# real-stanford/dgdm

Measured on AMD Instinct MI355X. Metric: guided samples/sec (full DDIM chain), higher is better.
Workload: dtype f32_split_f16x3; 1 GPU; 3d_guided BASELINE configs[2] (configs[3] at 8 GPUs): B=32 G=45 P=5 R=36000 sub_bs=512 N=512 T=15/S=5, fresh object per pair; contraction_flag=f32, fingers_per_pair=32, denoise_steps=5, rows_per_cond_fn=36000, cond_fn_per_chain_step=1, eps_net_form=f32_f16x3 batched, parallelism=pairs-sharded x1

## Files before the change

dgdm_amd/csrc/guidance_api.hip:

```cpp
#include "common.h"
#include "models.h"
#include <algorithm>
#include <cmath>
#include <cstring>
#include <unordered_map>
#include <atomic>
#include <thread>

using namespace dgdm;

namespace {

std::vector<float> linspace_f32(float start, float end, int steps) {
    std::vector<float> v(steps);
    if (steps == 1) { v[0] = start; return v; }
    const float step = (end - start) / (float)(steps - 1);
    const int half = steps / 2;
    for (int i = 0; i < steps; ++i) v[i] = i < half ? start + step * (float)i : end - step * (float)(steps - i - 1);
    return v;
}

struct ObjectTables {
    const float *xyz = nullptr;
    const int   *fps1 = nullptr;
    const int   *fps2 = nullptr;
    const int   *flags = nullptr;
    DevBuf Z;
    bool   fast_ok = false;
    int *crowded = nullptr, *clist = nullptr;
    DevBuf M0, cl2, cnt2;
    DevBuf cl2s;
    DevBuf cl2o;
    DevBuf pcf;
    DevBuf X, X16;
    bool   has_x = false, has_x16 = false;
    int    ncr = 0;
    DevBuf Z16, M0_16;
    bool   has16 = false;
};

struct PoseGrid {
    DevBuf tab, tiled;
    DevBuf pmax;
    int cells = 0, tiles_per_b = 0;
    int64_t rows = 0;
};

}

struct DgdmGuidance {
    DgdmDynamics *m = nullptr;
    DgdmGuidanceConfig cfg{};
    int B = 0;
    PoseGrid grid, sweep;
    DevBuf objpart;
    DevBuf objtmp;
    std::vector<std::unique_ptr<ObjectTables>> tables;
    bool bf16 = false;
    bool f32_mfma = false;
    static constexpr int NBUILD = 3;
    DevBuf pool_crowded, pool_clist, pool_off, pool_pairs, pool_rank, pool_F1, pool_U;
    DevBuf pool_xyz, pool_fps1, pool_fps2, pool_flags, pool_ncr;
    DevBuf pool_fps1t;
    DevBuf tmpY[NBUILD], tmpL2[NBUILD], vlist;
    DevBuf tmpShare[NBUILD];
    hipStream_t bstream[NBUILD] = {};
    hipEvent_t bev[NBUILD] = {}, bstart = nullptr, pooled = nullptr, ldone = nullptr;
    DevBuf V, genc, atab, chainbias, timepart, ttmp, ttmp64, partial, objdev, objidx, xobj, xobj16, starts, order, xchains, todo, groupoff;
    DevBuf loopx[2], loopeps, loopgrad, loopxrep, loopts;
    DevBuf loopeps1;
    DevBuf loopkeys;
    std::vector<uint64_t> loopkeys_host;
    DevBuf loopcond, loopx2, loopeps2;
    DevBuf scorelogits;
    DevBuf valobj;
    DevBuf sweep_ori, rollstate, rolllogits, rolltiles, rollpmax;
    const float *rowfield = nullptr;
    int rowfield_chains = 0;
    DevBuf pos_lin, goalspecs;
    DevBuf labelx, labelcounts, labelsums, labelfinal, labelfirst, labelleft, labelobj;
    int rolltiles_chains = 0;
    DevBuf xidx, xidxchains, xtabptrs;
    bool xtab_enabled = true;
    int xtab_policy = 0;
    int grads_since_set = 0;
    static constexpr int XTAB_AFTER = 5;
    int l2_gather_mode = 0;
    int xobj_mode = 0;
    int n_objects = 0;
    bool force_slow_xobj = false;
    void *pinned = nullptr; size_t pinned_bytes = 0; hipEvent_t pinned_ev = nullptr;
    int64_t todo_capacity = 0;
    int *ro_host = nullptr; size_t ro_ints = 0; hipEvent_t ro_ev = nullptr; bool ro_pending = false;
    int finish_objects();
    hipStream_t cstream = nullptr; hipEvent_t up_ready = nullptr, up_consumed = nullptr; bool consumed_recorded = false;
    int serial = 0;
    bool tables_off_stream() const { return !(serial & 3) && !prof_on(); }
    bool eps_beside() const { return !(serial & 5) && !prof_on(); }
    bool hoist_x_only() const { return !(serial & 1) && !prof_on(); }
    bool built_off_stream = false, join_pending = false, built_once = false;
    hipStream_t joined_stream = nullptr;
    hipEvent_t fork_ev = nullptr, side_ev = nullptr;
    int join_tables(hipStream_t s) {
        if (!built_off_stream || (!join_pending && s == joined_stream)) return DGDM_OK;
        DGDM_HIP_CHECK(hipStreamWaitEvent(s, ro_ev, 0));
        join_pending = false; joined_stream = s;
        return DGDM_OK;
    }
    int side_stream(hipStream_t *side) {
        if (!bstream[0]) DGDM_HIP_CHECK(hipStreamCreateWithFlags(&bstream[0], hipStreamNonBlocking));
        if (!fork_ev) DGDM_HIP_CHECK(hipEventCreateWithFlags(&fork_ev, hipEventDisableTiming));
        if (!side_ev) DGDM_HIP_CHECK(hipEventCreateWithFlags(&side_ev, hipEventDisableTiming));
        *side = bstream[0];
        return DGDM_OK;
    }
    ~DgdmGuidance() {
        for (int i = 0; i < NBUILD; ++i)
            if (bstream[i]) (void)hipStreamSynchronize(bstream[i]);
        if (fork_ev) (void)hipEventDestroy(fork_ev);
        if (side_ev) (void)hipEventDestroy(side_ev);
        if (pinned) (void)hipHostFree(pinned);
        if (pinned_ev) (void)hipEventDestroy(pinned_ev);
        if (ro_host) (void)hipHostFree(ro_host);
        if (ro_ev) (void)hipEventDestroy(ro_ev);
        if (cstream) (void)hipStreamDestroy(cstream);
        if (up_ready) (void)hipEventDestroy(up_ready);
        if (up_consumed) (void)hipEventDestroy(up_consumed);
        for (int i = 0; i < NBUILD; ++i) {
            if (bstream[i]) (void)hipStreamDestroy(bstream[i]);
            if (bev[i]) (void)hipEventDestroy(bev[i]);
        }
        if (bstart) (void)hipEventDestroy(bstart);
        if (ldone) (void)hipEventDestroy(ldone);
        if (pooled) (void)hipEventDestroy(pooled);
    }
    int build_pose_table(const std::vector<float> &ori, const std::vector<float> &pos, PoseGrid *dst, hipStream_t s);
    void set_grid(dgdm::TrunkParams *p, const PoseGrid &g, int n_chains) const;
    int check_objects(const int *oidx, int n_chains) const;
    bool tables_wanted() const { return xtab_enabled && !force_slow_xobj && xobj_mode == 0; }
    int common_pre(const float *x_dev, float t_scaled, const int *objidx_host, int n_chains, hipStream_t s);
    int upload_starts(const int64_t *starts_host, int n_chains, int64_t rows, hipStream_t s, bool need_order = true, int n_calls = 1,
                      int64_t call_stride = 0);
    int ensure_rows(int n_chains, int64_t rows_per_chain);
    int use_xtab(const int *objidx_host, int n_chains, int64_t rows, bool want16, hipStream_t s);
    int build_object(int oi, int slot, hipStream_t s);
    int build_xtab(int oi, hipStream_t s);
    int run_xobj(const int *objidx_host, int n_chains, int64_t rows, bool want16, bool *used16, bool *via_tab, hipStream_t s);
    struct Embedded {
        bool tab = false, used16 = false;
        int64_t rows_per_chain = 0;
        void point(dgdm::TrunkParams *p, const DgdmGuidance &g, int call, int64_t rows_per_call) const;
    };
    int embed_rows(const int *objidx_host, int n_chains, const int64_t *starts_host, int64_t rows_per_call, int n_calls, int64_t call_stride,
                   bool want16, Embedded *e, hipStream_t s);
    int embed(const int *objidx_host, int n_chains, const int64_t *starts_host, int n_calls, int64_t call_stride, Embedded *e, hipStream_t s);
    int trunk_front(int kind, const float *x_dev, int timestep, const int *objidx_host, const int64_t *starts_host, int n_chains, const Embedded *emb,
                    int call, dgdm::TrunkParams *p, hipStream_t s, bool pre_done = false);
};

int DgdmGuidance::build_pose_table(const std::vector<float> &ori, const std::vector<float> &pos, PoseGrid *dst, hipStream_t s) {
    const int n = (int)ori.size(), W1 = m->W1;
    dst->cells = n; dst->tiles_per_b = (n + 31) / 32; dst->rows = (int64_t)B * n;
    DevBuf d_ori, d_pos, d_emb;
    int rc;
    if ((rc = d_ori.upload(ori.data(), sizeof(float) * n))) return rc;
    if ((rc = d_pos.upload(pos.data(), sizeof(float) * 2 * n))) return rc;
    if ((rc = d_emb.alloc(sizeof(float) * 27 * n))) return rc;
    if ((rc = dst->tab.alloc(sizeof(float) * (size_t)W1 * n))) return rc;
    if ((rc = pose_embed(d_ori.as<float>(), d_pos.as<float>(), d_emb.as<float>(), n, s))) return rc;
    if ((rc = linear64(d_emb.as<float>(), nullptr, 27, m->blob64.at(m->off64.w1p_wt), nullptr, nullptr, 1, nullptr, dst->tab.as<float>(), W1, n, 27, W1, ACT_NONE, s))) return rc;
    if ((rc = dst->tiled.alloc(sizeof(float) * (size_t)W1 * dst->tiles_per_b * 32))) return rc;
    if ((rc = tile_table(dst->tab.as<float>(), n, W1, dst->tiled.as<float>(), s))) return rc;
    DGDM_HIP_CHECK(hipStreamSynchronize(s));
    return DGDM_OK;
}

void DgdmGuidance::set_grid(TrunkParams *p, const PoseGrid &g, int n_chains) const {
    p->Atab = atab.as<float>(); p->Ptab = g.tab.as<float>(); p->PtabT = g.tiled.as<float>(); p->Pmax = g.pmax.as<float>();
    p->B = B; p->C = g.cells; p->tiles_per_b = g.tiles_per_b; p->ntiles = n_chains * B * g.tiles_per_b; p->R = g.rows;
    p->xstride = g.rows;
}

int DgdmGuidance::check_objects(const int *oidx, int n_chains) const {
    DGDM_REQUIRE(n_objects > 0, DGDM_EINVAL, "dgdm_guidance_set_objects has not been called");
    for (int i = 0; i < n_chains; ++i)
        DGDM_REQUIRE(oidx[i] >= 0 && oidx[i] < n_objects, DGDM_EINVAL, "chain %d refers to object %d of %d", i, oidx[i], n_objects);
    return DGDM_OK;
}

extern "C" int dgdm_guidance_create(DgdmGuidance **out, DgdmDynamics *model, const DgdmGuidanceConfig *cfg) {
    DGDM_REQUIRE(out && model && cfg, DGDM_EINVAL, "dgdm_guidance_create: null argument");
    DGDM_REQUIRE(cfg->batch > 0 && cfg->grid_size > 0 && cfg->num_pos > 0 && cfg->max_chains > 0 && cfg->num_train_timesteps > 0,
                 DGDM_EINVAL, "dgdm_guidance_create: bad config");
    DGDM_REQUIRE(cfg->max_chains <= DGDM_MAX_CHAINS, DGDM_EINVAL, "max_chains %d > %d", cfg->max_chains, DGDM_MAX_CHAINS);
    if (model->kind == 3) {
        DGDM_REQUIRE(cfg->sub_batch_size > 0, DGDM_EINVAL, "3-D guidance needs sub_batch_size (it partitions the FPS start draws)");
        DGDM_REQUIRE(cfg->num_object_points > 0 && cfg->num_object_points <= 1024, DGDM_EINVAL, "object clouds of %d points unsupported (1..1024)", cfg->num_object_points);
    } else {
        DGDM_REQUIRE(2 * cfg->num_object_points == model->object_ch, DGDM_EINVAL, "2*num_object_points (%d) != object_ch (%d)", 2 * cfg->num_object_points, model->object_ch);
    }
    std::unique_ptr<DgdmGuidance> g(new DgdmGuidance());
    g->m = model; g->cfg = *cfg;
    g->B = cfg->batch;
    if (const char *e = getenv("DGDM_SERIAL_STEP")) g->serial = atoi(e);
    const int G = cfg->grid_size, P = cfg->num_pos, C = G * P * P;
    const std::vector<float> lo = linspace_f32(cfg->ori_lo, cfg->ori_hi, G), lp = linspace_f32(-1.f, 1.f, P);
    std::vector<float> ori(C), pos(2 * (size_t)C);
    for (int gi = 0; gi < G; ++gi)
        for (int a = 0; a < P; ++a)
            for (int b = 0; b < P; ++b) {
                const int c = (gi * P + a) * P + b;
                ori[c] = lo[gi]; pos[2 * c] = lp[a]; pos[2 * c + 1] = lp[b];
            }
    int rc;
    if ((rc = g->build_pose_table(ori, pos, &g->grid, nullptr))) return rc;
    {
        std::vector<float> tab((size_t)C * model->W1), mx(C, 0.f);
        DGDM_HIP_CHECK(hipMemcpy(tab.data(), g->grid.tab.p, tab.size() * sizeof(float), hipMemcpyDeviceToHost));
        for (int c = 0; c < C; ++c)
            for (int j = 0; j < model->W1; ++j) mx[c] = std::max(mx[c], std::fabs(tab[(size_t)c * model->W1 + j]));
        if ((rc = g->grid.pmax.upload(mx.data(), mx.size() * sizeof(float)))) return rc;
    }
    std::vector<float> pos0(2 * (size_t)G, 0.f);
    if ((rc = g->build_pose_table(lo, pos0, &g->sweep, nullptr))) return rc;
    if ((rc = g->sweep_ori.upload(lo.data(), lo.size() * sizeof(float)))) return rc;
    if ((rc = g->pos_lin.upload(lp.data(), lp.size() * sizeof(float)))) return rc;
    const int W1 = model->W1, nc = cfg->max_chains;
    const size_t rows = (size_t)nc * g->B;
    const int64_t R = g->grid.rows;
    if ((rc = g->V.alloc(rows * 256 * 8)) || (rc = g->genc.alloc(rows * 256 * 8)) || (rc = g->atab.alloc(rows * W1 * 4)) ||
        (rc = g->chainbias.alloc((size_t)nc * W1 * 8)) || (rc = g->timepart.alloc((size_t)W1 * 8)) || (rc = g->ttmp.alloc(768 * 4)) ||
        (rc = g->ttmp64.alloc(512 * 8)) ||
        (rc = g->partial.alloc(rows * g->grid.tiles_per_b * W1 * 4)) || (rc = g->objdev.alloc(sizeof(TrunkObjective) * nc)) ||
        (rc = g->objidx.alloc(sizeof(int) * nc)))
        return rc;
    if (model->kind == 2) {
        if ((rc = g->objpart.alloc((size_t)std::max(1, cfg->max_objects) * W1 * 8))) return rc;
    } else {
        if ((rc = g->starts.alloc((size_t)nc * R * 2 * sizeof(int))) ||
            (rc = g->order.alloc((size_t)nc * R * sizeof(int))) || (rc = g->xchains.alloc(sizeof(XobjChain) * nc)) ||
            (rc = g->todo.alloc(((size_t)nc * R + 1) * sizeof(int))))
            return rc;
        g->todo_capacity = (int64_t)nc * R;
        g->pinned_bytes = ((size_t)nc * R * 3 + (size_t)nc * (cfg->num_object_points + 1)) * sizeof(int);
        if ((rc = g->groupoff.alloc((size_t)nc * (cfg->num_object_points + 1) * sizeof(int))) || (rc = g->xidx.alloc((size_t)nc * R * sizeof(int))) ||
            (rc = g->xidxchains.alloc(sizeof(XidxChain) * nc)) || (rc = g->xtabptrs.alloc(sizeof(void *) * nc)))
            return rc;
        DGDM_HIP_CHECK(hipHostMalloc(&g->pinned, g->pinned_bytes, hipHostMallocDefault));
        DGDM_HIP_CHECK(hipEventCreateWithFlags(&g->pinned_ev, hipEventDisableTiming));
    }
    *out = g.release();
    return DGDM_OK;
}

extern "C" void dgdm_guidance_destroy(DgdmGuidance *g) { delete g; }

extern "C" int dgdm_guidance_set_contraction_dtype(DgdmGuidance *g, int dtype) {
    DGDM_REQUIRE(g, DGDM_EINVAL, "dgdm_guidance_set_contraction_dtype: null handle");
    DGDM_REQUIRE(dtype >= DGDM_DTYPE_F32 && dtype <= DGDM_DTYPE_F32_F16X3, DGDM_EINVAL,
                 "contraction dtype %d unsupported (0 = f32 (default form), 1 = bf16, 2 = f32 on the float32 MFMA, 3 = f32 as 3 f16 products = the default form)", dtype);
    g->bf16 = dtype == DGDM_DTYPE_BF16;
    g->f32_mfma = dtype == DGDM_DTYPE_F32_MFMA;
    return DGDM_OK;
}

extern "C" int dgdm_guidance_debug_fps_path(DgdmGuidance *g, int force_per_row, int32_t *out_fast_ok) {
    DGDM_REQUIRE(g, DGDM_EINVAL, "dgdm_guidance_debug_fps_path: null handle");
    g->force_slow_xobj = force_per_row == 1;
    g->xobj_mode = force_per_row == 2 ? 2 : 0;
    g->l2_gather_mode = force_per_row == 4 ? 1 : 0;
    g->xtab_enabled = force_per_row == 0 || force_per_row == 4 || force_per_row == 5;
    g->xtab_policy = force_per_row == 5 ? 1 : 0;
    if (force_per_row == 3) g->xobj_mode = 0;
    if (out_fast_ok) {
        int rc = g->finish_objects();
        if (rc) return rc;
        for (int i = 0; i < g->n_objects && i < (int)g->tables.size(); ++i) out_fast_ok[i] = g->tables[i]->fast_ok ? 1 : 0;
    }
    return DGDM_OK;
}
__global__ void partials_true_units_kernel(float *p, const float *unit, size_t n, int W1) {
    const size_t i = (size_t)blockIdx.x * blockDim.x + threadIdx.x;
    if (i < n) p[i] *= unit[i % W1];
}
extern "C" int dgdm_guidance_debug_partials(DgdmGuidance *g, int n_chains, float *out_dev, int32_t *tiles_per_finger, int32_t *width, void *stream) {
    DGDM_REQUIRE(g && n_chains > 0 && n_chains <= g->cfg.max_chains, DGDM_EINVAL, "dgdm_guidance_debug_partials: bad argument");
    if (tiles_per_finger) *tiles_per_finger = g->grid.tiles_per_b;
    if (width) *width = g->m->W1;
    if (out_dev) {
        const size_t n = (size_t)n_chains * g->B * g->grid.tiles_per_b * g->m->W1;
        DGDM_HIP_CHECK(hipMemcpyAsync(out_dev, g->partial.p, n * sizeof(float), hipMemcpyDeviceToDevice, (hipStream_t)stream));
        hipLaunchKernelGGL(partials_true_units_kernel, dim3((unsigned)((n + 255) / 256)), dim3(256), 0, (hipStream_t)stream, out_dev, g->m->z1_unit.as<float>(), n, g->m->W1);
        DGDM_HIP_CHECK(hipGetLastError());
    }
    return DGDM_OK;
}
extern "C" int64_t dgdm_guidance_rows(const DgdmGuidance *g) { return g ? g->grid.rows : 0; }
extern "C" int64_t dgdm_guidance_starts_per_call(const DgdmGuidance *g) { return (g && g->m->kind == 3) ? 2 * g->grid.rows : 0; }

int DgdmGuidance::build_object(int oi, int slot, hipStream_t s) {
    const int N = cfg.num_object_points;
    ObjectTables &t = *tables[oi];
    const PnWeights w = m->pn();
    int rc;
    if ((rc = t.Z.alloc((size_t)N * N * 256 * 4)) ||
        (rc = t.M0.alloc((size_t)N * 256 * 4)) || (rc = t.cl2.alloc((size_t)N * 128 * sizeof(int))) || (rc = t.cnt2.alloc((size_t)N * sizeof(int))) ||
        (rc = t.cl2s.alloc((size_t)N * 128 * sizeof(int))) || (rc = t.cl2o.alloc((size_t)N * 256 * sizeof(unsigned short))) ||
        (rc = t.pcf.alloc((size_t)N * 512 * sizeof(int))))
        return rc;
    t.has16 = bf16;
    if (bf16 && ((rc = t.Z16.alloc((size_t)N * N * 128 * 4)) || (rc = t.M0_16.alloc((size_t)N * 128 * 4)))) return rc;
    uint32_t *z16 = bf16 ? t.Z16.as<uint32_t>() : nullptr;
    DevBuf &tY = tmpY[slot], &tL2 = tmpL2[slot];
    if ((rc = tY.alloc((size_t)N * N * 256 * 4)) || (rc = tL2.alloc((size_t)N * N * 256 * 4))) return rc;
    const float *xyz = t.xyz;
    const int *off = pool_off.as<int>() + (size_t)oi * (N + 1), *pairs = pool_pairs.as<int>() + (size_t)oi * N * N;
    const short *rank = pool_rank.as<short>() + (size_t)oi * N * N;
    const char *U = static_cast<const char *>(pool_U.p) + (size_t)oi * N * 128 * (bf16 ? 4 : 8);
    if (bf16) {
        if ((rc = pn_pairs(xyz, N, reinterpret_cast<const float *>(U), w, pairs, off, tY.as<float>(), tY.as<uint32_t>(), s))) return rc;
        if ((rc = pn_l2(xyz, N, w, t.fps1, vlist.as<int>(), N, tY.as<float>(), tL2.as<float>(), t.clist, t.clist + N,
                        off, rank, true, s, l2_gather_mode ? 0 : 1))) return rc;
        if ((rc = pn_z16(xyz, N, N, w, tL2.as<uint32_t>(), t.Z.as<float>(), z16, t.clist, t.clist + N, s))) return rc;
    } else {
        const PnWeights64 w64 = m->pn64();
        if ((rc = pn_pairs64(xyz, N, reinterpret_cast<const double *>(U), w64, pairs, off, tY.as<float>(), s))) return rc;
        const bool shared = !l2_gather_mode && N <= 512;
        L2Share sh{};
        if (shared) {
            const size_t NN = (size_t)N * N;
            if ((rc = tmpShare[slot].alloc(NN * 64 + NN + NN * sizeof(short) + NN * sizeof(int) + (2 * (size_t)N + 4) * sizeof(int)))) return rc;
            char *b = static_cast<char *>(tmpShare[slot].p);
            sh.sel = reinterpret_cast<unsigned char *>(b); b += NN * 64;
            sh.items = reinterpret_cast<int *>(b); b += NN * sizeof(int);
            sh.coff = reinterpret_cast<int *>(b); b += N * sizeof(int);
            sh.ccnt = reinterpret_cast<int *>(b); b += N * sizeof(int);
            sh.nitems = reinterpret_cast<int *>(b); b += 4 * sizeof(int);
            sh.rep = reinterpret_cast<short *>(b); b += NN * sizeof(short);
            sh.cnt = reinterpret_cast<unsigned char *>(b);
            sh.fps1t = pool_fps1t.as<uint4>() + (size_t)oi * N * 64;
        }
        if ((rc = pn_l2(xyz, N, w, t.fps1, vlist.as<int>(), N, tY.as<float>(), tL2.as<float>(), t.clist, t.clist + N,
                        off, rank, false, s, shared ? 1 : 0, shared ? &sh : nullptr))) return rc;
        if ((rc = pn_z64(xyz, N, N, w64, tL2.as<float>(), t.Z.as<float>(), t.clist, t.clist + N, s, sh.items, sh.nitems))) return rc;
        if (shared && N > 1 && (rc = pn_zfill(N, N, t.Z.as<float>(), t.clist, t.clist + N, sh.rep, s))) return rc;
    }
    if ((rc = pn_m0(t.fps2, t.crowded, N, t.Z.as<float>(), t.M0.as<float>(), t.cl2.as<int>(), t.cnt2.as<int>(), z16,
                    bf16 ? t.M0_16.as<uint32_t>() : nullptr, t.clist, t.clist + N, t.cl2s.as<int>(), t.cl2o.as<unsigned short>(), s))) return rc;
    if ((rc = pn_pcf(t.fps1, t.cnt2.as<int>(), t.flags, N, t.pcf.as<int>(), s))) return rc;
    t.has_x = t.has_x16 = false;
    return xtab_policy == 1 ? build_xtab(oi, s) : DGDM_OK;
}

int DgdmGuidance::build_xtab(int oi, hipStream_t s) {
    const int N = cfg.num_object_points;
    ObjectTables &t = *tables[oi];
    if (N < 128) return DGDM_OK;
    const bool b16 = t.has16;
    int rc;
    if (b16) { if ((rc = t.X16.alloc((size_t)N * N * 128 * 4))) return rc; }
    else if ((rc = t.X.alloc((size_t)N * N * 256 * 4))) return rc;
    XtabObj xo{};
    xo.xyz = t.xyz; xo.fps1 = t.fps1; xo.Z = t.Z.as<float>(); xo.M0 = t.M0.as<float>();
    xo.Z16 = b16 ? t.Z16.as<uint32_t>() : nullptr; xo.M0_16 = b16 ? t.M0_16.as<uint32_t>() : nullptr;
    xo.clist = t.clist; xo.ncr = t.clist + N; xo.cl2s = t.cl2s.as<int>(); xo.cnt2 = t.cnt2.as<int>(); xo.flags = t.flags;
    xo.crowded = t.crowded; xo.X = b16 ? nullptr : t.X.as<float>(); xo.X16 = b16 ? t.X16.as<uint32_t>() : nullptr; xo.N = N;
    if ((rc = pn_xtab(xo, b16, s))) return rc;
    (b16 ? t.has_x16 : t.has_x) = true;
    return DGDM_OK;
}

extern "C" int dgdm_guidance_set_objects(DgdmGuidance *g, const float *objects_dev, int n_objects, void *stream) {
    DGDM_REQUIRE(g && objects_dev && n_objects > 0, DGDM_EINVAL, "dgdm_guidance_set_objects: bad argument");
    DGDM_REQUIRE(n_objects <= std::max(1, g->cfg.max_objects), DGDM_EINVAL, "%d objects > max_objects %d", n_objects, g->cfg.max_objects);
    hipStream_t s = (hipStream_t)stream;
    int rc;
    prof_begin(s, DGDM_STAGE_TABLES);
    if (g->m->kind == 2) {
        if ((rc = g->objtmp.alloc((size_t)n_objects * 512 * 8))) return rc;
        if ((rc = g->m->object_part_2d64(objects_dev, g->objtmp.as<double>(), g->objpart.as<double>(), n_objects, s))) return rc;
        prof_end(s, DGDM_STAGE_TABLES, 0.0);
    } else {
        while ((int)g->tables.size() < n_objects) g->tables.emplace_back(new ObjectTables());
        const int N = g->cfg.num_object_points;
        if (g->vlist.bytes < (size_t)N * sizeof(int)) {
            std::vector<int> v(N);
            for (int i = 0; i < N; ++i) v[i] = i;
            if ((rc = g->vlist.upload(v.data(), sizeof(int) * N))) return rc;
        }
        const int nb = std::min<int>(DgdmGuidance::NBUILD, n_objects);
        const bool off = g->tables_off_stream();
        const int ns = off ? std::max(nb, 2) : nb;
        if (!off && (rc = g->join_tables(s))) return rc;
        if (!g->bstart) DGDM_HIP_CHECK(hipEventCreateWithFlags(&g->bstart, hipEventDisableTiming));
        if (!g->ldone) DGDM_HIP_CHECK(hipEventCreateWithFlags(&g->ldone, hipEventDisableTiming));
        for (int i = 0; i < ns; ++i) {
            if (!g->bstream[i]) DGDM_HIP_CHECK(hipStreamCreateWithFlags(&g->bstream[i], hipStreamNonBlocking));
            if (!g->bev[i]) DGDM_HIP_CHECK(hipEventCreateWithFlags(&g->bev[i], hipEventDisableTiming));
        }
        const size_t no = (size_t)n_objects;
        if ((rc = g->pool_xyz.alloc(no * N * 3 * 4)) || (rc = g->pool_fps1.alloc(no * N * 512 * sizeof(int))) ||
            (rc = g->pool_fps2.alloc(no * N * 128 * sizeof(int))) || (rc = g->pool_flags.alloc(no * N * sizeof(int))) ||
            (rc = g->pool_ncr.alloc(no * sizeof(int))) || (rc = g->pool_crowded.alloc(no * N * sizeof(int))) ||
            (rc = g->pool_clist.alloc(no * (N + 1) * sizeof(int))) || (rc = g->pool_off.alloc(no * (N + 1) * sizeof(int))) ||
            (rc = g->pool_pairs.alloc(no * N * N * sizeof(int))) || (rc = g->pool_rank.alloc(no * N * N * sizeof(short))) ||
            (rc = g->pool_F1.alloc(no * N * 128 * 8)) || (rc = g->pool_U.alloc(no * N * 128 * 8)) ||
            (rc = g->pool_fps1t.alloc(no * N * 64 * sizeof(uint4))))
            return rc;
        if (!g->pooled) DGDM_HIP_CHECK(hipEventCreateWithFlags(&g->pooled, hipEventDisableTiming));
        DGDM_HIP_CHECK(hipMemcpyAsync(g->pool_xyz.p, objects_dev, no * N * 3 * 4, hipMemcpyDeviceToDevice, s));
        DGDM_HIP_CHECK(hipEventRecord(g->pooled, s));
        hipStream_t fs = s;
        if (off) {
            fs = g->bstream[ns - 1];
            for (int i = 1; i < ns; ++i) {
                DGDM_HIP_CHECK(hipStreamWaitEvent(g->bstream[i], g->pooled, 0));
                if (g->built_once) DGDM_HIP_CHECK(hipStreamWaitEvent(g->bstream[i], g->ro_ev, 0));
            }
        }
        if ((rc = pn_fps_tables(g->pool_xyz.as<float>(), N, N, g->pool_fps1.as<int>(), g->pool_fps2.as<int>(), g->pool_flags.as<int>(), fs, n_objects)))
            return rc;
        if (!g->bf16 && !g->l2_gather_mode && N <= 512 &&
            (rc = pn_fps_transpose(g->pool_fps1.as<int>(), N, g->pool_fps1t.as<uint4>(), fs, n_objects))) return rc;
        DGDM_HIP_CHECK(hipEventRecord(g->bstart, fs));
        for (int i = 0; i < n_objects; ++i) {
            ObjectTables &t = *g->tables[i];
            t.xyz = g->pool_xyz.as<float>() + (size_t)i * N * 3; t.fps1 = g->pool_fps1.as<int>() + (size_t)i * N * 512;
            t.fps2 = g->pool_fps2.as<int>() + (size_t)i * N * 128; t.flags = g->pool_flags.as<int>() + (size_t)i * N;
            t.crowded = g->pool_crowded.as<int>() + (size_t)i * N; t.clist = g->pool_clist.as<int>() + (size_t)i * (N + 1);
        }
        {
            hipStream_t ls = g->bstream[0];
            DGDM_HIP_CHECK(hipStreamWaitEvent(ls, g->pooled, 0));
            const PnWeights w = g->m->pn();
            if ((rc = pn_crowd(g->pool_xyz.as<float>(), N, w, g->pool_crowded.as<int>(), g->pool_clist.as<int>(), g->pool_clist.as<int>() + N,
                               g->pool_off.as<int>(), g->pool_pairs.as<int>(), g->pool_rank.as<short>(), ls, g->pool_ncr.as<int>(), n_objects)))
                return rc;
            if (g->bf16) {
                if ((rc = pn_sa1(g->pool_xyz.as<float>(), N, w, g->pool_F1.as<float>(), ls, n_objects))) return rc;
                if ((rc = linear(g->pool_F1.as<float>(), 128, w.sa2_wf_t, w.sa2_b0, nullptr, 1, g->pool_U.as<float>(), 128, n_objects * N, 128, 128,
                                 ACT_NONE, false, ls))) return rc;
            } else {
                const PnWeights64 w64 = g->m->pn64();
                if ((rc = pn_sa1_64(g->pool_xyz.as<float>(), N, w.r1sq, w64, g->pool_F1.as<double>(), ls, n_objects))) return rc;
                if ((rc = linear64(nullptr, g->pool_F1.as<double>(), 128, w64.sa2_wf_t, w64.sa2_b0, nullptr, 1, g->pool_U.as<double>(), nullptr, 128,
                                   n_objects * N, 128, 128, ACT_NONE, ls))) return rc;
            }
            DGDM_HIP_CHECK(hipEventRecord(g->ldone, ls));
        }
        for (int i = 0; i < nb; ++i) {
            DGDM_HIP_CHECK(hipStreamWaitEvent(g->bstream[i], g->bstart, 0));
            DGDM_HIP_CHECK(hipStreamWaitEvent(g->bstream[i], g->ldone, 0));
        }
        for (int i = 0; i < n_objects; ++i)
            if ((rc = g->build_object(i, i % nb, g->bstream[i % nb]))) return rc;
        hipStream_t es = off ? g->bstream[0] : s;
        for (int i = off ? 1 : 0; i < nb; ++i) {
            DGDM_HIP_CHECK(hipEventRecord(g->bev[i], g->bstream[i]));
            DGDM_HIP_CHECK(hipStreamWaitEvent(es, g->bev[i], 0));
        }
        prof_end(s, DGDM_STAGE_TABLES, 0.0);
        const size_t need = no * N + no;
        if (need > g->ro_ints) {
            if (g->ro_host) DGDM_HIP_CHECK(hipHostFree(g->ro_host));
            g->ro_host = nullptr;
            DGDM_HIP_CHECK(hipHostMalloc(reinterpret_cast<void **>(&g->ro_host), need * sizeof(int), hipHostMallocDefault));
            g->ro_ints = need;
        }
        if (!g->ro_ev) DGDM_HIP_CHECK(hipEventCreateWithFlags(&g->ro_ev, hipEventDisableTiming));
        DGDM_HIP_CHECK(hipMemcpyAsync(g->ro_host, g->pool_flags.p, sizeof(int) * no * N, hipMemcpyDeviceToHost, es));
        DGDM_HIP_CHECK(hipMemcpyAsync(g->ro_host + no * N, g->pool_ncr.p, sizeof(int) * no, hipMemcpyDeviceToHost, es));
        DGDM_HIP_CHECK(hipEventRecord(g->ro_ev, es));
        g->ro_pending = true;
        g->built_once = true; g->built_off_stream = off; g->join_pending = off;
    }
    g->n_objects = n_objects;
    g->grads_since_set = 0;
    return DGDM_OK;
}

int DgdmGuidance::common_pre(const float *x_dev, float t_scaled, const int *objidx_host, int n_chains, hipStream_t s) {
    const int rows = n_chains * B, W1 = m->W1;
    int rc;
    if ((rc = m->gripper_forward64(x_dev, m->L, V.as<double>(), genc.as<double>(), rows, s))) return rc;
    if ((rc = m->time_part64(t_scaled, ttmp.as<float>(), ttmp64.as<double>(), timepart.as<double>(), s))) return rc;
    if (m->kind == 2) {
        DGDM_HIP_CHECK(hipMemcpyAsync(objidx.p, objidx_host, sizeof(int) * n_chains, hipMemcpyHostToDevice, s));
        if ((rc = gather_add64(objpart.as<double>(), objidx.as<int>(), timepart.as<double>(), chainbias.as<double>(), n_chains, W1, s))) return rc;
        return linear64(nullptr, genc.as<double>(), 256, m->blob64.at(m->off64.w1c_wt), nullptr, chainbias.as<double>(), B, nullptr, atab.as<float>(), W1, rows, 256, W1,
                        ACT_NONE, s);
    }
    return linear64(nullptr, genc.as<double>(), 256, m->blob64.at(m->off64.w1c_wt), timepart.as<double>(), nullptr, 1, nullptr, atab.as<float>(), W1, rows, 256, W1,
                    ACT_NONE, s);
}

int DgdmGuidance::finish_objects() {
    if (!ro_pending) return DGDM_OK;
    DGDM_HIP_CHECK(hipEventSynchronize(ro_ev));
    const int N = cfg.num_object_points;
    for (int i = 0; i < n_objects; ++i) {
        bool ok = N >= 128;
        for (int k = 0; k < N; ++k) ok = ok && ro_host[(size_t)i * N + k] == 0;
        tables[i]->fast_ok = ok;
        tables[i]->ncr = ro_host[(size_t)n_objects * N + i];
    }
    ro_pending = false;
    return DGDM_OK;
}

int DgdmGuidance::ensure_rows(int n_chains, int64_t rows_per_chain) {
    const int N = cfg.num_object_points;
    const size_t nr = (size_t)n_chains * rows_per_chain;
    int rc;
    if ((rc = starts.alloc(nr * 2 * sizeof(int))) || (rc = order.alloc(nr * sizeof(int))) ||
        (rc = todo.alloc((nr + 1) * sizeof(int))) || (rc = xidx.alloc(nr * sizeof(int))))
        return rc;
    todo_capacity = (int64_t)nr;
    const size_t need = (nr * 3 + (size_t)n_chains * (N + 1)) * sizeof(int);
    if (need > pinned_bytes) {
        if (pinned) { DGDM_HIP_CHECK(hipEventSynchronize(pinned_ev)); DGDM_HIP_CHECK(hipHostFree(pinned)); pinned = nullptr; pinned_bytes = 0; }
        DGDM_HIP_CHECK(hipHostMalloc(&pinned, need, hipHostMallocDefault));
        pinned_bytes = need;
    }
    return DGDM_OK;
}

int DgdmGuidance::upload_starts(const int64_t *starts_host, int n_chains, int64_t rows, hipStream_t s, bool need_order, int n_calls,
                                int64_t call_stride) {
    const int N = cfg.num_object_points;
    const int64_t sb = cfg.sub_batch_size;
    const int64_t rt = rows * n_calls;
    int rc;
    DGDM_REQUIRE(!need_order || rt < ((int64_t)1 << 22), DGDM_EINVAL, "%lld rows per chain in one gather launch (limit 4194303)", (long long)rt);
    if ((rc = ensure_rows(n_chains, rt))) return rc;
    DGDM_HIP_CHECK(hipEventSynchronize(pinned_ev));
    int *dst = static_cast<int *>(pinned);
    int *ord = dst + (size_t)n_chains * 2 * rt;
    int *goff = ord + (size_t)n_chains * rt;
    std::atomic<int> bad{0};
    auto work = [&](int c0, int c1) {
        std::vector<int> cnt(N + 1), cnt2(513), tmp;
        for (int c = c0; c < c1; ++c) {
            int *d = dst + (size_t)c * 2 * rt;
            for (int k = 0; k < n_calls; ++k) {
                const int64_t *src = starts_host + (size_t)k * call_stride + (size_t)c * 2 * rows;
                int *dk = d + 2 * (size_t)k * rows;
                for (int64_t r0 = 0; r0 < rows; r0 += sb) {
                    const int64_t n = std::min(sb, rows - r0);
                    const int64_t *s1 = src + 2 * r0, *s2 = s1 + n;
                    for (int64_t i = 0; i < n; ++i) {
                        const int64_t a = s1[i], b = s2[i];
                        if (!(a >= 0 && a < N && b >= 0 && b < 512)) { bad.store(1); return; }
                        dk[2 * (r0 + i)] = (int)a; dk[2 * (r0 + i) + 1] = (int)b;
                    }
                }
            }
            if (!need_order) continue;
            int *o = ord + (size_t)c * rt;
            tmp.resize((size_t)rt);
            std::fill(cnt2.begin(), cnt2.end(), 0);
            for (int64_t r = 0; r < rt; ++r) ++cnt2[d[2 * r + 1] + 1];
            for (int k = 0; k < 512; ++k) cnt2[k + 1] += cnt2[k];
            for (int64_t r = 0; r < rt; ++r) tmp[cnt2[d[2 * r + 1]]++] = (int)r;
            std::fill(cnt.begin(), cnt.end(), 0);
            for (int64_t r = 0; r < rt; ++r) ++cnt[d[2 * r] + 1];
            for (int k = 0; k < N; ++k) cnt[k + 1] += cnt[k];
            memcpy(goff + (size_t)c * (N + 1), cnt.data(), sizeof(int) * (N + 1));
            for (int64_t i = 0; i < rt; ++i) { const int r = tmp[i]; o[cnt[d[2 * r]]++] = r | (d[2 * r + 1] << 22); }
        }
    };
    const int hw = (int)std::max(2u, std::thread::hardware_concurrency());
    const int nthreads = (int)std::min<int64_t>(std::min(16, hw / 2), std::max<int64_t>(1, std::min<int64_t>(n_chains, (int64_t)n_chains * rt / 65536)));
    if (nthreads <= 1) {
        work(0, n_chains);
    } else {
        std::vector<std::thread> pool;
        for (int t = 0; t < nthreads; ++t) pool.emplace_back(work, (int)((int64_t)n_chains * t / nthreads), (int)((int64_t)n_chains * (t + 1) / nthreads));
        for (auto &th : pool) th.join();
    }
    DGDM_REQUIRE(!bad.load(), DGDM_EINVAL, "FPS start out of range (sa1 must be in [0, %d), sa2 in [0, 512))", N);
    if (!cstream) {
        DGDM_HIP_CHECK(hipStreamCreateWithFlags(&cstream, hipStreamNonBlocking));
        DGDM_HIP_CHECK(hipEventCreateWithFlags(&up_ready, hipEventDisableTiming));
        DGDM_HIP_CHECK(hipEventCreateWithFlags(&up_consumed, hipEventDisableTiming));
    }
    if (consumed_recorded) DGDM_HIP_CHECK(hipStreamWaitEvent(cstream, up_consumed, 0));
    DGDM_HIP_CHECK(hipMemcpyAsync(starts.p, pinned, (size_t)n_chains * rt * 2 * sizeof(int), hipMemcpyHostToDevice, cstream));
    if (need_order) {
        DGDM_HIP_CHECK(hipMemcpyAsync(order.p, ord, (size_t)n_chains * rt * sizeof(int), hipMemcpyHostToDevice, cstream));
        DGDM_HIP_CHECK(hipMemcpyAsync(groupoff.p, goff, (size_t)n_chains * (N + 1) * sizeof(int), hipMemcpyHostToDevice, cstream));
    }
    DGDM_HIP_CHECK(hipEventRecord(pinned_ev, cstream));
    DGDM_HIP_CHECK(hipEventRecord(up_ready, cstream));
    DGDM_HIP_CHECK(hipStreamWaitEvent(s, up_ready, 0));
    return DGDM_OK;
}

int DgdmGuidance::use_xtab(const int *objidx_host, int n_chains, int64_t rows, bool want16, hipStream_t s) {
    std::vector<XidxChain> xc(n_chains);
    std::vector<const void *> base(n_chains);
    for (int i = 0; i < n_chains; ++i) {
        const ObjectTables &t = *tables[objidx_host[i]];
        xc[i].fps1 = t.fps1; xc[i].N = cfg.num_object_points; xc[i].m0_only = t.ncr == 0;
        base[i] = want16 ? (t.ncr == 0 ? (const void *)t.M0_16.p : (const void *)t.X16.p) : (t.ncr == 0 ? (const void *)t.M0.p : (const void *)t.X.p);
    }
    DGDM_HIP_CHECK(hipMemcpyAsync(xidxchains.p, xc.data(), sizeof(XidxChain) * n_chains, hipMemcpyHostToDevice, s));
    DGDM_HIP_CHECK(hipMemcpyAsync(xtabptrs.p, base.data(), sizeof(void *) * n_chains, hipMemcpyHostToDevice, s));
    return pn_xidx(xidxchains.as<XidxChain>(), starts.as<int>(), rows, n_chains, xidx.as<int>(), s);
}

int DgdmGuidance::run_xobj(const int *objidx_host, int n_chains, int64_t rows, bool want16, bool *used16, bool *via_tab, hipStream_t s) {
    *via_tab = false;
    std::vector<XobjChain> ch(n_chains);
    for (int i = 0; i < n_chains; ++i) {
        const ObjectTables &t = *tables[objidx_host[i]];
        ch[i].xyz = t.xyz; ch[i].fps1 = t.fps1; ch[i].slot_of_start = nullptr; ch[i].Z = t.Z.as<float>();
        ch[i].fps2 = t.fps2; ch[i].flags = t.flags; ch[i].crowded = t.crowded; ch[i].N = cfg.num_object_points;
        ch[i].M0 = t.M0.as<float>(); ch[i].cl2 = t.cl2.as<int>(); ch[i].cnt2 = t.cnt2.as<int>();
        ch[i].Z16 = t.has16 ? t.Z16.as<uint32_t>() : nullptr; ch[i].M0_16 = t.has16 ? t.M0_16.as<uint32_t>() : nullptr;
        want16 = want16 && t.has16;
    }
    {
        const size_t nrows = (size_t)n_chains * rows;
        int rc = want16 ? xobj16.alloc(nrows * 512) : xobj.alloc(nrows * 256 * 4);
        if (rc) return rc;
    }
    *used16 = want16;
    XobjParams xp{};
    xp.chains = xchains.as<XobjChain>(); xp.starts = starts.as<int>(); xp.order = order.as<int>(); xp.xobj = xobj.as<float>();
    xp.xobj16 = want16 ? xobj16.as<uint32_t>() : nullptr;
    xp.R = rows; xp.total_rows = rows * n_chains; xp.use_table = force_slow_xobj ? 0 : 1;
    xp.todo = todo.as<int>(); xp.todo_count = todo.as<int>() + todo_capacity; xp.todo_capacity = todo_capacity;
    bool all_fast = true;
    for (int i = 0; i < n_chains; ++i) all_fast = all_fast && tables[objidx_host[i]]->fast_ok;
    bool groups = !force_slow_xobj && xobj_mode == 0 && cfg.num_object_points >= 128;
    for (int i = 0; i < n_chains && groups; ++i) {
        const ObjectTables &t = *tables[objidx_host[i]];
        const int lpr = xobj_rows_lpr(t.ncr, want16);
        groups = lpr > 0 && want16 == t.has16;
        ch[i].clist = t.clist; ch[i].cl2s = t.cl2s.as<int>(); ch[i].cl2o = t.cl2o.as<unsigned short>(); ch[i].pcf = t.pcf.as<int>(); ch[i].ncr = t.ncr; ch[i].lpr = lpr;
    }
    DGDM_HIP_CHECK(hipMemcpyAsync(xchains.p, ch.data(), sizeof(XobjChain) * n_chains, hipMemcpyHostToDevice, s));
    if (groups) {
        const bool by_index = tables_wanted() && (want16 || !bf16);
        std::vector<int> rank;
        std::vector<XidxChain> xc(n_chains);
        std::vector<const void *> base(n_chains);
        for (int i = 0; i < n_chains; ++i) {
            const ObjectTables &t = *tables[objidx_host[i]];
            const bool m0_only = by_index && t.ncr == 0 && t.fast_ok;
            if (!m0_only) rank.push_back(i);
            xc[i].fps1 = m0_only ? t.fps1 : nullptr; xc[i].N = cfg.num_object_points; xc[i].m0_only = 1;
            base[i] = m0_only ? (want16 ? (const void *)t.M0_16.p : (const void *)t.M0.p)
                              : (want16 ? (const void *)(xobj16.as<uint32_t>() + (size_t)i * rows * 128) : (const void *)(xobj.as<float>() + (size_t)i * rows * 256));
        }
        xp.group_off = groupoff.as<int>(); xp.nchain = n_chains; xp.group_N = cfg.num_object_points; xp.use_table = 1;
        xp.total_items = (int)rank.size() * xp.group_N;
        std::stable_sort(rank.begin(), rank.end(), [&](int a, int b) { return ch[a].ncr > ch[b].ncr; });
        for (size_t i = 0; i < rank.size(); ++i) xp.chain_of_rank[i] = (unsigned char)rank[i];
        int rc = pn_xobj_groups(xp, s);
        if (rc || !by_index) return rc;
        *via_tab = true;
        DGDM_HIP_CHECK(hipMemcpyAsync(xidxchains.p, xc.data(), sizeof(XidxChain) * n_chains, hipMemcpyHostToDevice, s));
        DGDM_HIP_CHECK(hipMemcpyAsync(xtabptrs.p, base.data(), sizeof(void *) * n_chains, hipMemcpyHostToDevice, s));
        return pn_xidx(xidxchains.as<XidxChain>(), starts.as<int>(), rows, n_chains, xidx.as<int>(), s);
    }
    return pn_xobj(xp, all_fast, s);
}

int DgdmGuidance::embed_rows(const int *oidx, int n_chains, const int64_t *starts_host, int64_t rows_per_call, int n_calls, int64_t call_stride,
                             bool want16, Embedded *e, hipStream_t s) {
    bool tab = tables_wanted();
    for (int i = 0; i < n_chains && tab; ++i) tab = want16 ? tables[oidx[i]]->has_x16 : tables[oidx[i]]->has_x;
    const int64_t rt = rows_per_call * n_calls;
    int rc;
    if ((rc = join_tables(s))) return rc;
    if ((rc = upload_starts(starts_host, n_chains, rows_per_call, s, !tab, n_calls, call_stride))) return rc;
    if ((rc = finish_objects())) return rc;
    e->tab = tab; e->used16 = want16; e->rows_per_chain = rt;
    if ((rc = tab ? use_xtab(oidx, n_chains, rt, want16, s) : run_xobj(oidx, n_chains, rt, want16, &e->used16, &e->tab, s))) return rc;
    DGDM_HIP_CHECK(hipEventRecord(up_consumed, s));
    consumed_recorded = true;
    return DGDM_OK;
}

void DgdmGuidance::Embedded::point(TrunkParams *p, const DgdmGuidance &g, int call, int64_t rows_per_call) const {
    const size_t row0 = (size_t)call * rows_per_call;
    p->xstride = rows_per_chain;
    if (tab) {
        p->xidx = g.xidx.as<int>() + row0;
        if (used16) p->xtab16 = g.xtabptrs.as<const uint32_t *>();
        else p->xtab = g.xtabptrs.as<const float *>();
    } else {
        p->xobj = g.xobj.as<float>() + row0 * 256;
        p->xobj16 = used16 ? g.xobj16.as<uint32_t>() + row0 * 128 : nullptr;
    }
}

int DgdmGuidance::embed(const int *oidx, int n_chains, const int64_t *starts_host, int n_calls, int64_t call_stride, Embedded *e, hipStream_t s) {
    DGDM_REQUIRE(starts_host, DGDM_EINVAL, "3-D guidance needs the FPS start indices");
    int rc;
    if ((rc = join_tables(s))) return rc;
    prof_begin(s, DGDM_STAGE_XOBJ);
    if (tables_wanted()) {
        const bool crosses = grads_since_set <= XTAB_AFTER && grads_since_set + n_calls > XTAB_AFTER;
        grads_since_set += n_calls;
        if (crosses)
            for (int i = 0; i < n_objects; ++i) {
                ObjectTables &t = *tables[i];
                if (!(t.has16 ? t.has_x16 : t.has_x) && (rc = build_xtab(i, s))) return rc;
            }
    }
    if ((rc = embed_rows(oidx, n_chains, starts_host, grid.rows, n_calls, call_stride, bf16, e, s))) return rc;
    prof_end(s, DGDM_STAGE_XOBJ, 0.0);
    return DGDM_OK;
}

int DgdmGuidance::trunk_front(int kind, const float *x_dev, int timestep, const int *oidx, const int64_t *starts_host, int n_chains, const Embedded *emb,
                              int call, TrunkParams *pp, hipStream_t s, bool pre_done) {
    const float t_scaled = (float)timestep / (float)cfg.num_train_timesteps;
    int rc;
    if ((rc = check_objects(oidx, n_chains))) return rc;
    if (!pre_done) {
        prof_begin(s, DGDM_STAGE_GUIDE_MISC);
        if ((rc = common_pre(x_dev, t_scaled, oidx, n_chains, s))) return rc;
        prof_end(s, DGDM_STAGE_GUIDE_MISC, 0.0);
    }
    m->fill_trunk(pp);
    set_grid(pp, grid, n_chains);
    if (kind == 3) {
        Embedded own;
        if (!emb) {
            if ((rc = embed(oidx, n_chains, starts_host, 1, 0, &own, s))) return rc;
            emb = &own;
            call = 0;
        }
        emb->point(pp, *this, call, grid.rows);
    }
    return DGDM_OK;
}

static int check_objectives(const DgdmGuidance *g, const DgdmObjective *objectives, const float *rowcoef_dev, int n_chains) {
    for (int i = 0; i < n_chains; ++i) {
        const int u = objectives[i].use_rowcoef;
        DGDM_REQUIRE(u >= 0 && u <= DGDM_OBJ_ROWFIELD, DGDM_EINVAL, "chain %d: use_rowcoef %d (0, 1 or %d)", i, u, DGDM_OBJ_ROWFIELD);
        DGDM_REQUIRE(u != 1 || rowcoef_dev, DGDM_EINVAL, "chain %d uses rowcoef but rowcoef_dev is null", i);
        if (u == DGDM_OBJ_ROWFIELD) {
            DGDM_REQUIRE(g->rowfield, DGDM_EINVAL, "chain %d uses the row field but none is set (dgdm_guidance_set_row_field)", i);
            DGDM_REQUIRE(i < g->rowfield_chains, DGDM_EINVAL, "chain %d uses the row field, which was set for %d chains", i, g->rowfield_chains);
        }
    }
    return DGDM_OK;
}

static int guidance_grad(DgdmGuidance *g, int kind, const float *x_dev, int timestep, const DgdmObjective *objectives, const float *rowcoef_dev,
                         const int64_t *starts_host, int n_chains, float *grad_dev, hipStream_t s, const DgdmGuidance::Embedded *emb = nullptr,
                         int call = 0, bool pre_done = false) {
    DGDM_REQUIRE(g && x_dev && objectives && grad_dev, DGDM_EINVAL, "guidance_grad: null argument");
    if (g->m->kind != kind) { set_error("model type not supported: %d-D entry point on a %d-D model", kind, g->m->kind); return DGDM_EMODE; }
    DGDM_REQUIRE(n_chains > 0 && n_chains <= g->cfg.max_chains, DGDM_EINVAL, "n_chains %d outside 1..%d", n_chains, g->cfg.max_chains);
    int rc;
    if ((rc = check_objectives(g, objectives, rowcoef_dev, n_chains))) return rc;
    std::vector<int> oidx(n_chains);
    std::vector<TrunkObjective> tob(n_chains);
    for (int i = 0; i < n_chains; ++i) {
        oidx[i] = objectives[i].object;
        for (int j = 0; j < 3; ++j) { tob[i].lin[j] = objectives[i].lin[j]; tob[i].quad[j] = objectives[i].quad[j]; }
        tob[i].use_rowcoef = objectives[i].use_rowcoef; tob[i].pad = 0;
    }
    TrunkParams p;
    if ((rc = g->trunk_front(kind, x_dev, timestep, oidx.data(), starts_host, n_chains, emb, call, &p, s, pre_done))) return rc;
    DGDM_HIP_CHECK(hipMemcpyAsync(g->objdev.p, tob.data(), sizeof(TrunkObjective) * n_chains, hipMemcpyHostToDevice, s));
    p.obj = g->objdev.as<TrunkObjective>(); p.rowcoef = rowcoef_dev; p.rowfield = g->rowfield;
    p.partial = g->partial.as<float>();
    if (g->bf16) {
        g->m->fill_trunk_bf16(&p);
        if ((rc = trunk_bf16_launch(kind, p, s))) return rc;
    } else if (g->f32_mfma) {
        if ((rc = trunk_launch(kind, false, false, p, s))) return rc;
    } else {
        TrunkF16Scales sc;
        g->m->fill_trunk_f16(&p, &sc);
        if ((rc = trunk_f16l_launch(kind, TrunkF16Mode::Grad, p, sc, s))) return rc;
    }
    prof_begin(s, DGDM_STAGE_GUIDE_MISC);
    rc = dyn_post64(g->m->W1, g->partial.as<float>(), g->grid.tiles_per_b, g->m->blob64.at(g->m->off64.w1c_w), g->m->blob64.at(g->m->off64.g2_w),
                    g->m->blob64.at(g->m->off64.g0_w), g->V.as<double>(), grad_dev, n_chains * g->B, g->m->L, s);
    prof_end(s, DGDM_STAGE_GUIDE_MISC, 0.0);
    return rc;
}

extern "C" int dgdm_dyn2d_guidance_grad(DgdmGuidance *g, const float *x_dev, int timestep, const DgdmObjective *objectives,
                                        const float *rowcoef_dev, int n_chains, float *grad_dev, void *stream) {
    return guidance_grad(g, 2, x_dev, timestep, objectives, rowcoef_dev, nullptr, n_chains, grad_dev, (hipStream_t)stream);
}

extern "C" int dgdm_dyn3d_guidance_grad(DgdmGuidance *g, const float *x_dev, int timestep, const DgdmObjective *objectives,
                                        const float *rowcoef_dev, const int64_t *starts_host, int n_chains, float *grad_dev, void *stream) {
    return guidance_grad(g, 3, x_dev, timestep, objectives, rowcoef_dev, starts_host, n_chains, grad_dev, (hipStream_t)stream);
}

extern "C" int dgdm_guidance_set_row_field(DgdmGuidance *g, const float *field_dev, int n_chains, void *stream) {
    (void)stream;
    DGDM_REQUIRE(g, DGDM_EINVAL, "dgdm_guidance_set_row_field: null handle");
    if (!field_dev) { g->rowfield = nullptr; g->rowfield_chains = 0; return DGDM_OK; }
    DGDM_REQUIRE(n_chains > 0 && n_chains <= g->cfg.max_chains, DGDM_EINVAL, "dgdm_guidance_set_row_field: n_chains %d outside 1..%d", n_chains,
                 g->cfg.max_chains);
    g->rowfield = field_dev; g->rowfield_chains = n_chains;
    return DGDM_OK;
}

extern "C" int dgdm_guidance_goal_field(DgdmGuidance *g, const float *goals_dev, const DgdmGoalSpec *specs_host, int n_chains, float *field_dev,
                                        void *stream) {
    DGDM_REQUIRE(g && goals_dev && specs_host && field_dev, DGDM_EINVAL, "dgdm_guidance_goal_field: null argument");
    DGDM_REQUIRE(n_chains > 0 && n_chains <= g->cfg.max_chains, DGDM_EINVAL, "dgdm_guidance_goal_field: n_chains %d outside 1..%d", n_chains,
                 g->cfg.max_chains);
    hipStream_t s = (hipStream_t)stream;
    for (int i = 0; i < n_chains; ++i) {
        const DgdmGoalSpec &q = specs_host[i];
        DGDM_REQUIRE(q.ori_window > 0.f && q.ori_window <= 1.f, DGDM_EINVAL, "goal %d: ori_window %g outside (0, 1]", i, (double)q.ori_window);
        DGDM_REQUIRE(q.pos_window > 0.f && std::isfinite(q.pos_window), DGDM_EINVAL, "goal %d: pos_window %g is not a positive number", i, (double)q.pos_window);
        DGDM_REQUIRE(q.profile == 0 || q.profile == 1, DGDM_EINVAL, "goal %d: profile %d (0 sign, 1 linear)", i, q.profile);
        for (int j = 0; j < 3; ++j) DGDM_REQUIRE(std::isfinite(q.weight[j]), DGDM_EINVAL, "goal %d: weight %d is not finite", i, j);
    }
    std::vector<float> goals((size_t)n_chains * g->B * 3);
    DGDM_HIP_CHECK(hipMemcpyAsync(goals.data(), goals_dev, goals.size() * sizeof(float), hipMemcpyDeviceToHost, s));
    DGDM_HIP_CHECK(hipStreamSynchronize(s));
    for (size_t k = 0; k < goals.size(); ++k)
        DGDM_REQUIRE(std::isfinite(goals[k]), DGDM_EINVAL, "goal %d, finger %d: coordinate %d is not finite", (int)(k / ((size_t)g->B * 3)),
                     (int)(k / 3 % g->B), (int)(k % 3));
    int rc;
    if ((rc = g->goalspecs.alloc(sizeof(DgdmGoalSpec) * g->cfg.max_chains))) return rc;
    DGDM_HIP_CHECK(hipMemcpyAsync(g->goalspecs.p, specs_host, sizeof(DgdmGoalSpec) * n_chains, hipMemcpyHostToDevice, s));
    return goal_field_build(g->sweep_ori.as<float>(), g->pos_lin.as<float>(), goals_dev, g->goalspecs.as<DgdmGoalSpec>(), n_chains, g->B,
                            g->cfg.grid_size, g->cfg.num_pos, field_dev, s);
}

extern "C" int dgdm_guidance_score(DgdmGuidance *g, const float *x_dev, int timestep, const int32_t *object_of_chain, const int64_t *starts_host,
                                   const float thr[3], int n_chains, float *logits_dev, int32_t *counts_dev, float *sums_dev, void *stream) {
    DGDM_REQUIRE(g && x_dev && object_of_chain && thr && counts_dev && sums_dev, DGDM_EINVAL, "dgdm_guidance_score: null argument");
    DGDM_REQUIRE(!g->bf16, DGDM_EINVAL, "dgdm_guidance_score: the bf16 trunk has no forward-only form (contraction dtypes f32 / f32_f16x3 / f32_mfma)");
    hipStream_t s = (hipStream_t)stream;
    const int kind = g->m->kind;
    DGDM_REQUIRE(kind == 2 || starts_host, DGDM_EINVAL, "3-D scoring needs the FPS start indices");
    DGDM_REQUIRE(n_chains > 0 && n_chains <= g->cfg.max_chains, DGDM_EINVAL, "n_chains %d outside 1..%d", n_chains, g->cfg.max_chains);
    int rc;
    if (!logits_dev) {
        if ((rc = g->scorelogits.alloc((size_t)n_chains * g->grid.rows * 3 * sizeof(float)))) return rc;
        logits_dev = g->scorelogits.as<float>();
    }
    const std::vector<int> oidx(object_of_chain, object_of_chain + n_chains);
    TrunkParams p;
    if ((rc = g->trunk_front(kind, x_dev, timestep, oidx.data(), starts_host, n_chains, nullptr, 0, &p, s))) return rc;
    p.logits = logits_dev;
    if (g->f32_mfma) {
        if ((rc = trunk_launch(kind, false, true, p, s))) return rc;
    } else {
        TrunkF16Scales sc;
        g->m->fill_trunk_f16(&p, &sc);
        if ((rc = trunk_f16l_launch(kind, TrunkF16Mode::Forward, p, sc, s))) return rc;
    }
    return score_tally(logits_dev, n_chains, g->B, g->grid.cells, thr, counts_dev, sums_dev, s);
}

extern "C" int dgdm_guidance_objective_values(DgdmGuidance *g, const float *logits_dev, const DgdmObjective *objectives, const float *rowcoef_dev,
                                              int n_chains, double *values_dev, void *stream) {
    DGDM_REQUIRE(g && logits_dev && objectives && values_dev, DGDM_EINVAL, "dgdm_guidance_objective_values: null argument");
    DGDM_REQUIRE(n_chains > 0 && n_chains <= g->cfg.max_chains, DGDM_EINVAL, "n_chains %d outside 1..%d", n_chains, g->cfg.max_chains);
    int rc;
    if ((rc = check_objectives(g, objectives, rowcoef_dev, n_chains))) return rc;
    hipStream_t s = (hipStream_t)stream;
    std::vector<TrunkObjective> tob(n_chains);
    for (int i = 0; i < n_chains; ++i) {
        for (int j = 0; j < 3; ++j) { tob[i].lin[j] = objectives[i].lin[j]; tob[i].quad[j] = objectives[i].quad[j]; }
        tob[i].use_rowcoef = objectives[i].use_rowcoef; tob[i].pad = 0;
    }
    if ((rc = g->valobj.alloc(sizeof(TrunkObjective) * g->cfg.max_chains))) return rc;
    DGDM_HIP_CHECK(hipMemcpyAsync(g->valobj.p, tob.data(), sizeof(TrunkObjective) * n_chains, hipMemcpyHostToDevice, s));
    return objective_values_launch(logits_dev, g->valobj.as<TrunkObjective>(), rowcoef_dev, g->rowfield, n_chains, g->B, g->grid.cells, values_dev, s);
}

namespace {
__global__ void fill_i32_kernel(int *p, int v, int n) {
    const int i = blockIdx.x * blockDim.x + threadIdx.x;
    if (i < n) p[i] = v;
}
__global__ void repeat_rows_kernel(const float *__restrict__ src, float *__restrict__ dst, int64_t n_src, int reps) {
    const int64_t i = (int64_t)blockIdx.x * blockDim.x + threadIdx.x;
    if (i < n_src * reps) dst[i] = src[i % n_src];
}
__global__ void cfg_mix_kernel(const float *ec, const float *eu, float w, float *out, int64_t n) {
    const int64_t i = (int64_t)blockIdx.x * blockDim.x + threadIdx.x;
    if (i >= n) return;
    const float u = eu[i];
    out[i] = add_rn(u, mul_rn(w, sub_rn(ec[i], u)));
}
}

extern "C" int dgdm_cfg_mix(const float *eps_c_dev, const float *eps_u_dev, float w, float *out_dev, int64_t numel, void *stream) {
    DGDM_REQUIRE(eps_c_dev && eps_u_dev && out_dev && numel >= 0, DGDM_EINVAL, "dgdm_cfg_mix: bad argument");
    if (numel == 0) return DGDM_OK;
    hipLaunchKernelGGL(cfg_mix_kernel, dim3((unsigned)((numel + 255) / 256)), dim3(256), 0, (hipStream_t)stream, eps_c_dev, eps_u_dev, w, out_dev, numel);
    DGDM_HIP_CHECK(hipGetLastError());
    return DGDM_OK;
}

extern "C" int dgdm_guided_chains_run(DgdmUnet1d *unet, DgdmGuidance *g, const float *noise_dev, int n_chains, int n_grad,
                                      const DgdmObjective *objectives, const float *rowcoef_dev, const int64_t *starts_host,
                                      const int32_t *timesteps, const float *coef, const float *scales, int n_steps, float *x_out_dev,
                                      void *stream) {
    return dgdm_guided_chains_run_cond(unet, g, noise_dev, n_chains, n_grad, objectives, rowcoef_dev, starts_host, timesteps, coef, scales, n_steps, x_out_dev,
                                       nullptr, 0, 1.f, stream);
}

extern "C" int dgdm_guided_chains_run_cond(DgdmUnet1d *unet, DgdmGuidance *g, const float *noise_dev, int n_chains, int n_grad,
                                           const DgdmObjective *objectives, const float *rowcoef_dev, const int64_t *starts_host,
                                           const int32_t *timesteps, const float *coef, const float *scales, int n_steps, float *x_out_dev,
                                           const float *global_cond_dev, int64_t cond_chain_stride, float cfg_weight, void *stream) {
    return dgdm_guided_chains_run_bounded(unet, g, noise_dev, n_chains, n_grad, objectives, rowcoef_dev, starts_host, timesteps, coef, scales, n_steps, x_out_dev,
                                          global_cond_dev, cond_chain_stride, cfg_weight, nullptr, nullptr, stream);
}

extern "C" int dgdm_guided_chains_run_bounded(DgdmUnet1d *unet, DgdmGuidance *g, const float *noise_dev, int n_chains, int n_grad,
                                              const DgdmObjective *objectives, const float *rowcoef_dev, const int64_t *starts_host,
                                              const int32_t *timesteps, const float *coef, const float *scales, int n_steps, float *x_out_dev,
                                              const float *global_cond_dev, int64_t cond_chain_stride, float cfg_weight, const float *lo_dev,
                                              const float *hi_dev, void *stream) {
    return dgdm_guided_chains_run_noisy(unet, g, noise_dev, n_chains, n_grad, objectives, rowcoef_dev, starts_host, timesteps, coef, scales, n_steps, x_out_dev,
                                        global_cond_dev, cond_chain_stride, cfg_weight, lo_dev, hi_dev, nullptr, 0, nullptr, stream);
}

extern "C" int dgdm_guided_chains_run_noisy(DgdmUnet1d *unet, DgdmGuidance *g, const float *noise_dev, int n_chains, int n_grad,
                                            const DgdmObjective *objectives, const float *rowcoef_dev, const int64_t *starts_host,
                                            const int32_t *timesteps, const float *coef, const float *scales, int n_steps, float *x_out_dev,
                                            const float *global_cond_dev, int64_t cond_chain_stride, float cfg_weight, const float *lo_dev,
                                            const float *hi_dev, const float *eta_coef, uint64_t seed, const uint64_t *chain_keys, void *stream) {
    DGDM_REQUIRE(unet && g && noise_dev && objectives && timesteps && coef && scales && x_out_dev, DGDM_EINVAL, "dgdm_guided_chains_run: null argument");
    DGDM_REQUIRE(!lo_dev == !hi_dev, DGDM_EINVAL, "dgdm_guided_chains_run_bounded: lo and hi come together or not at all");
    DGDM_REQUIRE(n_chains > 0 && n_grad > 0 && n_chains * n_grad <= g->cfg.max_chains && n_steps > 0, DGDM_EINVAL,
                 "dgdm_guided_chains_run: %d chains x %d gradients outside 1..%d", n_chains, n_grad, g->cfg.max_chains);
    hipStream_t s = (hipStream_t)stream;
    const int B = g->B, L = g->m->L, kind = g->m->kind;
    const size_t per_chain = (size_t)B * L, nx = per_chain * n_chains, ng = nx * n_grad;
    DGDM_REQUIRE(kind == 2 || starts_host, DGDM_EINVAL, "3-D guidance needs the FPS start indices");
    const int gc = dgdm_unet1d_global_cond_dim(unet);
    DGDM_REQUIRE(gc == 0 || global_cond_dev, DGDM_EINVAL, "dgdm_guided_chains_run: the eps-net has global_cond_dim %d and needs a condition", gc);
    DGDM_REQUIRE(cfg_weight == cfg_weight && std::fabs(cfg_weight) <= 3.0e38f, DGDM_EINVAL, "dgdm_guided_chains_run: cfg_weight is not finite");
    const bool conditional = gc > 0;
    DGDM_REQUIRE(!conditional || cond_chain_stride == 0 || cond_chain_stride == (int64_t)B * gc, DGDM_EINVAL,
                 "dgdm_guided_chains_run: cond_chain_stride %lld is neither 0 (one [B][%d] block for all chains) nor B * gc = %lld", (long long)cond_chain_stride, gc,
                 (long long)B * gc);
    const bool per_chain_cond = conditional && cond_chain_stride != 0 && n_chains > 1;
    const int cfg = !conditional ? 1 : cfg_weight == 1.f ? 1 : cfg_weight == 0.f ? 0 : 2;
    int rc;
    if ((rc = check_objectives(g, objectives, rowcoef_dev, n_chains * n_grad))) return rc;
    bool noisy = false;
    for (int si = 0; eta_coef && si < n_steps; ++si) {
        const float sg = eta_coef[2 * si], dr = eta_coef[2 * si + 1];
        DGDM_REQUIRE(sg >= 0.f && sg <= 3.0e38f && dr == dr, DGDM_EINVAL, "dgdm_guided_chains_run_noisy: step %d has sigma %g, dir %g", si, (double)sg, (double)dr);
        noisy = noisy || sg != 0.f;
    }
    const uint64_t *keys_dev = nullptr;
    if (noisy) {
        std::vector<uint64_t> keys(n_chains);
        for (int c = 0; c < n_chains; ++c) keys[c] = chain_keys ? chain_keys[c] : (uint64_t)c;
        if (keys != g->loopkeys_host || !g->loopkeys.p) {
            g->loopkeys_host.clear();
            if ((rc = g->loopkeys.alloc(sizeof(uint64_t) * n_chains))) return rc;
            DGDM_HIP_CHECK(hipMemcpyAsync(g->loopkeys.p, keys.data(), sizeof(uint64_t) * n_chains, hipMemcpyHostToDevice, (hipStream_t)stream));
            DGDM_HIP_CHECK(hipStreamSynchronize((hipStream_t)stream));
            g->loopkeys_host = keys;
        }
        keys_dev = g->loopkeys.as<uint64_t>();
    }
    if ((rc = g->loopx[0].alloc(nx * 4)) || (rc = g->loopx[1].alloc(nx * 4)) || (rc = g->loopeps.alloc(nx * 4)) || (rc = g->loopgrad.alloc(ng * 4)) ||
        (rc = g->loopxrep.alloc(ng * 4)) || (rc = g->loopts.alloc((size_t)2 * n_chains * B * sizeof(int))))
        return rc;
    const size_t ncond = (size_t)n_chains * B * gc;
    const float *cond_rows = nullptr, *zero_rows = nullptr;
    if (conditional) {
        if ((rc = g->loopcond.alloc(2 * ncond * 4))) return rc;
        float *cr = g->loopcond.as<float>();
        if (cond_chain_stride == 0) hipLaunchKernelGGL(repeat_rows_kernel, dim3((unsigned)((ncond + 255) / 256)), dim3(256), 0, s, global_cond_dev, cr, (int64_t)B * gc, n_chains);
        else DGDM_HIP_CHECK(hipMemcpyAsync(cr, global_cond_dev, ncond * 4, hipMemcpyDeviceToDevice, s));
        DGDM_HIP_CHECK(hipMemsetAsync(cr + ncond, 0, ncond * 4, s));
        cond_rows = cr; zero_rows = cr + ncond;
        if (cfg == 2 && ((rc = g->loopx2.alloc(2 * nx * 4)) || (rc = g->loopeps2.alloc(2 * nx * 4)))) return rc;
    }
    hipLaunchKernelGGL(repeat_rows_kernel, dim3((unsigned)((nx + 255) / 256)), dim3(256), 0, s, noise_dev, g->loopx[0].as<float>(), (int64_t)per_chain, n_chains);
    bool same_scale = true;
    for (int c = 1; c < n_chains; ++c) same_scale = same_scale && scales[c] == scales[0];
    const int64_t spc = kind == 3 ? 2 * g->grid.rows : 0;
    DgdmGuidance::Embedded emb;
    std::vector<int> oidx(n_chains * n_grad);
    const int64_t call_stride = (int64_t)n_chains * n_grad * spc;
// ... 361 lines not shown
```

dgdm_amd/csrc/models.h:

```cpp
#pragma once
#include "common.h"
#include "blob.h"
#include "unet.h"
#include "trunk.h"
#include "pointnet.h"
#include "smallnet.h"
#include <memory>

struct DgdmUnet1d {
    dgdm::Blob blob;
    dgdm::UnetParams p;
    dgdm::DevBuf p_dev;
    dgdm::DevBuf w16;
    dgdm::DevBuf p16_dev;
    dgdm::DevBuf wf16;
    dgdm::DevBuf pf16_dev;
    int mode = 2;
    dgdm::UnetParams pf16;
    dgdm::DevBuf bws;
    int bws_B = 0, bws_L = 0;
    int batched_min = 768;
};

namespace dgdm {
struct DynOff {
    size_t g0_wt, g0_b, g0_w, g2_wt, g2_b, g2_w;
    size_t w1c_wt, w1c_w, w1p_wt, w1t_wt, b1, w1o_wt;
    size_t b2;
    size_t bf[8];
    size_t wfwd, wbwd;
    size_t fwd_floats, bwd_floats;
    size_t wout, bout;
    size_t te0_wt, te0_b, te2_wt, te2_b, oe0_wt, oe0_b, oe2_wt, oe2_b, tfreq;
    size_t sa1_w0t, sa1_b0, sa1_w1, sa1_b1, sa2_wf_t, sa2_b0, sa2_vx, sa2_w1_img, sa2_b1, sa3_wx, sa3_b;
};
struct DynOff64 {
    size_t g0_wt, g0_b, g0_w, g2_wt, g2_b, g2_w;
    size_t w1c_wt, w1c_w, w1p_wt, w1t_wt, b1, w1o_wt;
    size_t te0_wt, te0_b, te2_wt, te2_b, oe0_wt, oe0_b, oe2_wt, oe2_b;
    size_t sa1_w0t, sa1_b0, sa1_w1, sa1_b1, sa2_wf_t, sa2_b0, sa2_vx, sa2_w1_img, sa2_b1, sa3_w_img, sa3_wx, sa3_b;
};
}

struct DgdmDynamics {
    int kind = 0, L = 0, object_ch = 0, W1 = 256, n_mid = 7, thalf = 64;
    dgdm::Blob blob;
    dgdm::DynOff off{};
    dgdm::Blob64 blob64;
    dgdm::DynOff64 off64{};
    dgdm::DevBuf ws;
    dgdm::DevBuf ws2;
    dgdm::DevBuf w16;
    size_t fwd16_bytes = 0, bwd16_bytes = 0, sa3_16_offset = 0;
    dgdm::DevBuf wf16;
    size_t fwdh_bytes = 0, bwdh_bytes = 0;
    dgdm::TrunkF16Scales f16_scales{};
    dgdm::DevBuf z1_unit;

    void fill_trunk(dgdm::TrunkParams *p) const;
    void fill_trunk_f16(dgdm::TrunkParams *p, dgdm::TrunkF16Scales *sc) const;
    void fill_trunk_bf16(dgdm::TrunkParams *p) const;
    dgdm::PnWeights pn() const;
    int gripper_forward(const float *x, int ldx, float *V, float *genc, int rows, hipStream_t s) const;
    int time_part(const float *t_dev, float t_scalar, float *tmp, float *out, int rows, hipStream_t s) const;
    int object_part_2d(const float *obj, float *tmp, float *out, int n, bool accumulate, hipStream_t s) const;
    int gripper_forward64(const float *x, int ldx, double *V64, double *genc64, int rows, hipStream_t s) const;
    int time_part64(float t_scalar, float *tmp, double *tmp64, double *out64, hipStream_t s) const;
    int object_part_2d64(const float *obj, double *tmp64, double *out64, int n, hipStream_t s) const;
    dgdm::PnWeights64 pn64() const;
};
```

dgdm_amd/csrc/models_api.hip:

```cpp
#include "common.h"
#include <climits>
#include "blob.h"
#include "models.h"
#include <algorithm>
#include <cmath>
#include <cstring>

using namespace dgdm;

namespace {

template <class At>
std::vector<float> conv_image(int cout, int cin, const std::vector<int> &taps, At at) {
    const int mt = cout / 16, g = cin / 16, nt = (int)taps.size();
    std::vector<float> o((size_t)cout * cin * nt);
    for (int m = 0; m < mt; ++m)
        for (int t = 0; t < nt; ++t)
            for (int gg = 0; gg < g; ++gg)
                for (int lane = 0; lane < 64; ++lane)
                    for (int c = 0; c < 4; ++c)
                        o[((((size_t)m * nt + t) * g + gg) * 64 + lane) * 4 + c] = at(16 * m + (lane & 15), 16 * gg + 4 * (lane >> 4) + c, taps[t]);
    return o;
}

// ... 288 lines not shown
    const int mode = (m->mode == 2 && !unet_f16x3_fits(m->p, L)) ? 0 : m->mode;
    const bool batched = mode == 2 && m->batched_min > 0 && B >= m->batched_min && unet_batched_samples(m->pf16, L) > 0;
    return (mode == 1 ? DGDM_DTYPE_BF16 : mode == 2 ? DGDM_DTYPE_F32_F16X3 : DGDM_DTYPE_F32_MFMA) + (batched ? 16 : 0);
}

extern "C" int dgdm_unet1d_set_contraction_dtype(DgdmUnet1d *m, int dtype) {
    DGDM_REQUIRE(m, DGDM_EINVAL, "dgdm_unet1d_set_contraction_dtype: null handle");
    DGDM_REQUIRE(dtype >= DGDM_DTYPE_F32 && dtype <= DGDM_DTYPE_F32_F16X3, DGDM_EINVAL, "contraction dtype %d unsupported", dtype);
    m->mode = dtype == DGDM_DTYPE_BF16 ? 1 : dtype == DGDM_DTYPE_F32_MFMA ? 0 : 2;
    return DGDM_OK;
}

namespace {

std::vector<float> cols(const std::vector<float> &w, int rows, int ncols, int c0, int n) {
    std::vector<float> o((size_t)rows * n);
    for (int r = 0; r < rows; ++r)
        for (int c = 0; c < n; ++c) o[(size_t)r * n + c] = w[(size_t)r * ncols + c0 + c];
    return o;
}

std::vector<double> cols64(const std::vector<double> &w, int rows, int ncols, int c0, int n) {
    std::vector<double> o((size_t)rows * n);
    for (int r = 0; r < rows; ++r)
        for (int c = 0; c < n; ++c) o[(size_t)r * n + c] = w[(size_t)r * ncols + c0 + c];
    return o;
}

struct Split2 {
    std::vector<float> p[2];
    int K = 0, ew = 0;
    static float f16(float x) { const _Float16 h = (_Float16)x; return (float)h; }
    static uint16_t bits(float x) { const _Float16 h = (_Float16)x; uint16_t u; memcpy(&u, &h, 2); return u; }
    Split2(const float *src, int M, int K_) : K(K_) {
        float mx = 0.f;
        for (size_t i = 0; i < (size_t)M * K_; ++i) mx = std::max(mx, std::fabs(src[i]));
        int e = 0;
        if (mx > 0.f) std::frexp(mx, &e);
        ew = 13 - e;
        for (auto &v : p) v.resize((size_t)M * K_);
        for (size_t i = 0; i < (size_t)M * K_; ++i) {
            const float w = std::ldexp(src[i], ew), h = f16(w);
            p[0][i] = h; p[1][i] = f16(w - h);
        }
    }
    void emit(std::vector<uint16_t> &dst, int op, int ib, int s) const {
        for (int q = 0; q < 2; ++q)
            for (int lane = 0; lane < 64; ++lane) {
                const int i = lane & 31, hh = lane >> 5;
                for (int j = 0; j < 8; ++j) {
                    const int rr = 8 * s + j, f = (rr & 3) + 8 * (rr >> 2) + 4 * hh;
                    dst.push_back(bits(p[q][(size_t)(32 * op + i) * K + 32 * ib + f]));
                }
            }
    }
};
int f16_layer_stream(std::vector<uint16_t> &dst, const float *w ) {
    const Split2 sp(w, 256, 256);
    for (int ks = 0; ks < 16; ++ks)
        for (int pp = 0; pp < 4; ++pp)
            for (int blk = 2 * pp; blk < 2 * pp + 2; ++blk) sp.emit(dst, blk, ks / 2, ks % 2);
    return sp.ew;
}

std::vector<float> tfreqs(int half) {
    std::vector<float> f(half);
    const float l = -(float)std::log(10000.0);
    for (int i = 0; i < half; ++i) f[i] = expf(l * (float)i / (float)half);
    return f;
}

struct TrunkEquil {
    std::vector<std::vector<int>> e;
    std::vector<std::vector<char>> dead;
    int W1 = 0;
    static std::string lin(int l) { return "linears." + std::to_string(3 * l); }
    static std::string bn(int l) { return "linears." + std::to_string(3 * l + 1); }
    int out_of(int l) const { return l == 0 ? W1 : 256; }
    int build(const StateDict &sd, int W1_, int IN1) {
        W1 = W1_;
        e.assign(8, {});
        dead.assign(8, {});
        double A = 1.0;
        for (int l = 0; l < 8; ++l) {
            const int out = out_of(l), in = l == 0 ? IN1 : out_of(l - 1);
            Folded64 f;
            const int rc = fold_linear64(sd, lin(l), bn(l), out, in, &f);
            if (rc) return rc;
            std::vector<int> re(out, INT_MIN);
            std::vector<double> mw(out, 0.0);
            std::vector<char> zero_row(out, 1);
            int top = INT_MIN;
            for (int j = 0; j < out; ++j) {
                for (int k = 0; k < in; ++k) {
                    const double w = std::fabs(f.w[(size_t)j * in + k]);
                    if (l && dead[l - 1][k]) continue;
                    if (std::isfinite(w)) mw[j] = std::max(mw[j], l ? std::ldexp(w, -e[l - 1][k]) : w);
                }
                zero_row[j] = mw[j] == 0.0;
                const double b = std::fabs(f.b[j]);
                const double mx = std::max(mw[j], (A > 0.0 && std::isfinite(b)) ? b / A : 0.0);
                if (mx > 0.0) { std::frexp(mx, &re[j]); top = std::max(top, re[j]); }
            }
            dead[l].assign(out, 0);
            for (int j = 0; j < out; ++j) dead[l][j] = zero_row[j] && f.b[j] <= 0.0;
            e[l].assign(out, 0);
            double An = 0.0;
            for (int j = 0; j < out; ++j) {
                if (re[j] != INT_MIN && !dead[l][j]) e[l][j] = std::min(top - re[j], 60);
                if (!dead[l][j] && std::isfinite(f.b[j])) An = std::max(An, std::ldexp(std::max(std::fabs(f.b[j]), mw[j] * A), e[l][j]));
            }
            A = An;
        }
        return DGDM_OK;
    }
    template <class F>
    int apply(F *f, int l) const {
        for (int j = 0; j < f->out; ++j) {
            const int ej = l < 8 ? e[l][j] : 0;
            for (int k = 0; k < f->in; ++k)
                f->w[(size_t)j * f->in + k] = (l && dead[l - 1][k]) ? 0 : std::ldexp(f->w[(size_t)j * f->in + k], ej - (l ? e[l - 1][k] : 0));
            f->b[j] = std::ldexp(f->b[j], ej);
        }
        return DGDM_OK;
    }
    int fold(const StateDict &sd, int l, int out, int in, Folded *dst) const {
        const int rc = l < 8 ? fold_linear(sd, lin(l), bn(l), out, in, dst) : fold_linear(sd, "output", "", out, in, dst);
        return rc ? rc : apply(dst, l);
    }
    int fold64(const StateDict &sd, int l, int out, int in, Folded64 *dst) const {
        const int rc = l < 8 ? fold_linear64(sd, lin(l), bn(l), out, in, dst) : fold_linear64(sd, "output", "", out, in, dst);
        return rc ? rc : apply(dst, l);
    }
};

}

extern "C" int dgdm_dynamics_create(DgdmDynamics **out, int kind, const DgdmTensor *tensors, int n_tensors, int params_ch, int object_ch) {
    DGDM_REQUIRE(out && tensors, DGDM_EINVAL, "dgdm_dynamics_create: null argument");
    if (kind != 2 && kind != 3) { set_error("model type not supported: kind %d", kind); return DGDM_EMODE; }
    DGDM_REQUIRE(params_ch > 0 && params_ch <= 256, DGDM_EINVAL, "params_ch %d unsupported", params_ch);
    StateDict sd(tensors, n_tensors);
    std::unique_ptr<DgdmDynamics> m(new DgdmDynamics());
    m->kind = kind; m->L = params_ch; m->object_ch = object_ch; m->W1 = kind == 3 ? 512 : 256;
    const int W = 256, W1 = m->W1, IN1 = 3 * W + 27;
    Blob &bl = m->blob;
    int rc;
    TrunkEquil eq;
    if ((rc = eq.build(sd, W1, IN1))) return rc;
    if (getenv("DGDM_NO_EQUILIBRATION")) for (int l = 0; l < 8; ++l) { std::fill(eq.e[l].begin(), eq.e[l].end(), 0); std::fill(eq.dead[l].begin(), eq.dead[l].end(), 0); }
    {
        std::vector<float> u(W1);
        for (int j = 0; j < W1; ++j) u[j] = std::ldexp(1.0f, eq.e[0][j]);
        if ((rc = m->z1_unit.upload(u.data(), u.size() * sizeof(float)))) return rc;
    }
    Folded g0, g2, l1, lout;
    if ((rc = fold_linear(sd, "gripper_encoder.0", "", W, params_ch, &g0))) return rc;
    if ((rc = fold_linear(sd, "gripper_encoder.2", "", W, W, &g2))) return rc;
    if ((rc = eq.fold(sd, 0, W1, IN1, &l1))) return rc;
    if ((rc = eq.fold(sd, 8, 3, W, &lout))) return rc;
    DynOff &o = m->off;
    std::vector<float> fwd, bwd_tail;
    std::vector<uint16_t> fwd16, bwd16_tail, sa3_img16;
    const size_t E16 = 64 * 8;
    o.g0_wt = bl.add(transpose(g0.w.data(), W, params_ch)); o.g0_b = bl.add(g0.b); o.g0_w = bl.add(g0.w);
    o.g2_wt = bl.add(transpose(g2.w.data(), W, W)); o.g2_b = bl.add(g2.b); o.g2_w = bl.add(g2.w);
    const std::vector<float> w1o = cols(l1.w, W1, IN1, 0, W), w1c = cols(l1.w, W1, IN1, W, W), w1p = cols(l1.w, W1, IN1, 2 * W, 27),
                             w1t = cols(l1.w, W1, IN1, 2 * W + 27, W);
    o.w1c_wt = bl.add(transpose(w1c.data(), W1, W)); o.w1c_w = bl.add(w1c);
    o.w1p_wt = bl.add(transpose(w1p.data(), W1, 27));
    o.w1t_wt = bl.add(transpose(w1t.data(), W1, W));
    o.b1 = bl.add(l1.b);
    o.wout = bl.add(lout.w); o.bout = bl.add(lout.b);
    int first_mid = 1;
    if (kind == 2) {
        o.w1o_wt = bl.add(transpose(w1o.data(), W1, W));
        Folded t0, t2, e0, e2;
        if ((rc = fold_linear(sd, "time_encoder.0", "", W, W / 2, &t0))) return rc;
        if ((rc = fold_linear(sd, "time_encoder.2", "", W, W, &t2))) return rc;
        if ((rc = fold_linear(sd, "object_encoder.0", "", W, object_ch, &e0))) return rc;
        if ((rc = fold_linear(sd, "object_encoder.2", "", W, W, &e2))) return rc;
        o.te0_wt = bl.add(transpose(t0.w.data(), W, W / 2)); o.te0_b = bl.add(t0.b);
        o.te2_wt = bl.add(transpose(t2.w.data(), W, W)); o.te2_b = bl.add(t2.b);
        o.oe0_wt = bl.add(transpose(e0.w.data(), W, object_ch)); o.oe0_b = bl.add(e0.b);
        o.oe2_wt = bl.add(transpose(e2.w.data(), W, W)); o.oe2_b = bl.add(e2.b);
        o.tfreq = bl.add(tfreqs(W / 4));
        m->thalf = W / 4;
    } else {
        Folded l2;
        if ((rc = eq.fold(sd, 1, W, W1, &l2))) return rc;
        o.b2 = bl.add(l2.b);
        const std::vector<float> i1 = pack_chain(w1o.data(), W1, W), i2 = pack_chain(l2.w.data(), W, W1);
        const size_t E = 64 * 4;
        for (int blk = 0; blk < 16; ++blk) {
            fwd.insert(fwd.end(), i1.begin() + (size_t)blk * 32 * E, i1.begin() + (size_t)(blk + 1) * 32 * E);
            for (int op = 0; op < 8; ++op)
                fwd.insert(fwd.end(), i2.begin() + (size_t)((op * 16 + blk) * 4) * E, i2.begin() + (size_t)((op * 16 + blk) * 4 + 4) * E);
        }
        bwd_tail = pack_chain(transpose(l2.w.data(), W, W1).data(), W1, W);
        {
            const std::vector<uint16_t> j1 = pack_chain_bf16(w1o.data(), W1, W), j2 = pack_chain_bf16(l2.w.data(), W, W1);
            auto put_z = [&](int kb) { fwd16.insert(fwd16.end(), j1.begin() + (size_t)kb * 16 * E16, j1.begin() + (size_t)(kb + 1) * 16 * E16); };
            auto put_l2 = [&](int kb) {
                for (int op = 0; op < 8; ++op)
                    fwd16.insert(fwd16.end(), j2.begin() + (size_t)((op * 16 + kb) * 2) * E16, j2.begin() + (size_t)((op * 16 + kb) * 2 + 2) * E16);
            };
            put_z(0);
            for (int kb = 1; kb < 16; ++kb) { put_z(kb); put_l2(kb - 1); }
            put_l2(15);
            bwd16_tail = pack_chain_bf16(transpose(l2.w.data(), W, W1).data(), W1, W);
        }
        o.tfreq = bl.add(tfreqs(W / 2));
        m->thalf = W / 2;
        first_mid = 2;
        Folded a0, a1, b0, b1, c0;
        if ((rc = fold_linear(sd, "object_encoder.sa1.mlp_convs.0", "object_encoder.sa1.mlp_bns.0", 64, 3, &a0))) return rc;
        if ((rc = fold_linear(sd, "object_encoder.sa1.mlp_convs.1", "object_encoder.sa1.mlp_bns.1", 128, 64, &a1))) return rc;
        if ((rc = fold_linear(sd, "object_encoder.sa2.mlp_convs.0", "object_encoder.sa2.mlp_bns.0", 128, 131, &b0))) return rc;
        if ((rc = fold_linear(sd, "object_encoder.sa2.mlp_convs.1", "object_encoder.sa2.mlp_bns.1", 256, 128, &b1))) return rc;
        if ((rc = fold_linear(sd, "object_encoder.sa3.mlp_convs.0", "object_encoder.sa3.mlp_bns.0", 256, 259, &c0))) return rc;
        o.sa1_w0t = bl.add(transpose(a0.w.data(), 64, 3)); o.sa1_b0 = bl.add(a0.b);
        o.sa1_w1 = bl.add(a1.w); o.sa1_b1 = bl.add(a1.b);
        o.sa2_wf_t = bl.add(transpose(cols(b0.w, 128, 131, 3, 128).data(), 128, 128)); o.sa2_b0 = bl.add(b0.b);
        o.sa2_vx = bl.add(transpose(cols(b0.w, 128, 131, 0, 3).data(), 128, 3));
        o.sa2_w1_img = bl.add(pack_chain(b1.w.data(), 256, 128)); o.sa2_b1 = bl.add(b1.b);
        sa3_img16 = pack_chain_bf16(cols(c0.w, 256, 259, 3, 256).data(), 256, 256);
        o.sa3_wx = bl.add(transpose(cols(c0.w, 256, 259, 0, 3).data(), 256, 3)); o.sa3_b = bl.add(c0.b);
    }
    m->n_mid = 8 - first_mid;
    std::vector<std::vector<float>> bwd_imgs;
    std::vector<std::vector<uint16_t>> bwd16_imgs;
    for (int i = 0; i < m->n_mid; ++i) {
        const int li = 3 * (first_mid + i);
        Folded f;
        if ((rc = eq.fold(sd, li / 3, W, W, &f))) return rc;
        const std::vector<float> fi = pack_chain(f.w.data(), W, W);
        fwd.insert(fwd.end(), fi.begin(), fi.end());
        o.bf[i] = bl.add(f.b);
        bwd_imgs.push_back(pack_chain(transpose(f.w.data(), W, W).data(), W, W));
        const std::vector<uint16_t> f16 = pack_chain_bf16(f.w.data(), W, W);
        fwd16.insert(fwd16.end(), f16.begin(), f16.end());
        bwd16_imgs.push_back(pack_chain_bf16(transpose(f.w.data(), W, W).data(), W, W));
    }
    {
        std::vector<float> wo((size_t)32 * W, 0.f), wot((size_t)W * 32, 0.f);
        for (int j = 0; j < 3; ++j)
            for (int k = 0; k < W; ++k) { wo[(size_t)j * W + k] = lout.w[(size_t)j * W + k]; wot[(size_t)k * 32 + j] = lout.w[(size_t)j * W + k]; }
        const std::vector<uint16_t> o16 = pack_chain_bf16(wo.data(), 32, W), ot16 = pack_chain_bf16(wot.data(), W, 32);
        fwd16.insert(fwd16.end(), o16.begin(), o16.end());
        std::vector<uint16_t> bwd16(ot16);
        for (int i = m->n_mid - 1; i >= 0; --i) bwd16.insert(bwd16.end(), bwd16_imgs[i].begin(), bwd16_imgs[i].end());
        bwd16.insert(bwd16.end(), bwd16_tail.begin(), bwd16_tail.end());
        m->fwd16_bytes = fwd16.size() * 2; m->bwd16_bytes = bwd16.size() * 2;
        fwd16.insert(fwd16.end(), bwd16.begin(), bwd16.end());
        m->sa3_16_offset = fwd16.size() * 2;
        fwd16.insert(fwd16.end(), sa3_img16.begin(), sa3_img16.end());
        if ((rc = m->w16.upload(fwd16.data(), fwd16.size() * 2))) return rc;
    }
    {
        std::vector<uint16_t> fs, bs;
        TrunkF16Scales &sc = m->f16_scales;
        sc = TrunkF16Scales{};
        Folded l2;
        if (kind == 3) {
            if ((rc = eq.fold(sd, 1, W, W1, &l2))) return rc;
            const std::vector<float> w1o3 = cols(l1.w, W1, IN1, 0, W);
            const Split2 s1(w1o3.data(), W1, W);
            const Split2 s2(l2.w.data(), W, W1);
            sc.ew_l1 = s1.ew;
            sc.ew_l2 = s2.ew;
            float n1 = 0.f;
            for (int j = 0; j < W1; ++j) {
                double a = 0.0;
                for (int k = 0; k < W; ++k) a += std::fabs((double)w1o3[(size_t)j * W + k]);
                n1 = std::max(n1, (float)(a * (1.0 + 1e-6)));
            }
            sc.l1_norm1 = n1;
            for (int kb = 0; kb < 16; ++kb) {
                for (int ks = 0; ks < 16; ++ks) s1.emit(fs, kb, ks / 2, ks % 2);
                for (int pp = 0; pp < 4; ++pp)
                    for (int sx = 0; sx < 2; ++sx)
                        for (int blk = 2 * pp; blk < 2 * pp + 2; ++blk) s2.emit(fs, blk, kb, sx);
            }
        }
        std::vector<std::vector<uint16_t>> back;
        for (int i = 0; i < m->n_mid; ++i) {
            const int li = 3 * (first_mid + i);
            Folded f;
            if ((rc = eq.fold(sd, li / 3, W, W, &f))) return rc;
            sc.ew_mid[i] = f16_layer_stream(fs, f.w.data());
            back.emplace_back();
            const int et = f16_layer_stream(back.back(), transpose(f.w.data(), W, W).data());
            DGDM_REQUIRE(et == sc.ew_mid[i], DGDM_EINVAL, "f16 split: a matrix and its transpose disagree about their scale");
        }
        for (int i = m->n_mid - 1; i >= 0; --i) bs.insert(bs.end(), back[i].begin(), back[i].end());
        if (kind == 3) {
            const std::vector<float> w2t = transpose(l2.w.data(), W, W1);
            const Split2 st(w2t.data(), W1, W);
            DGDM_REQUIRE(st.ew == sc.ew_l2, DGDM_EINVAL, "f16 split: layer 2 and its transpose disagree about their scale");
            for (int kb = 0; kb < 16; ++kb)
                for (int ks = 0; ks < 16; ++ks) st.emit(bs, kb, ks / 2, ks % 2);
        }
        m->fwdh_bytes = fs.size() * 2; m->bwdh_bytes = bs.size() * 2;
        fs.insert(fs.end(), bs.begin(), bs.end());
        if ((rc = m->wf16.upload(fs.data(), fs.size() * 2))) return rc;
    }
    std::vector<float> bwd;
    for (int i = m->n_mid - 1; i >= 0; --i) bwd.insert(bwd.end(), bwd_imgs[i].begin(), bwd_imgs[i].end());
    bwd.insert(bwd.end(), bwd_tail.begin(), bwd_tail.end());
    o.wfwd = bl.add(fwd); o.fwd_floats = fwd.size();
    o.wbwd = bl.add(bwd); o.bwd_floats = bwd.size();
    if ((rc = bl.upload())) return rc;
    {
        Blob64 &b6 = m->blob64;
        DynOff64 &q = m->off64;
        Folded64 h0, h2, k1;
        if ((rc = fold_linear64(sd, "gripper_encoder.0", "", W, params_ch, &h0))) return rc;
        if ((rc = fold_linear64(sd, "gripper_encoder.2", "", W, W, &h2))) return rc;
        if ((rc = eq.fold64(sd, 0, W1, IN1, &k1))) return rc;
        q.g0_wt = b6.add(transpose64(h0.w.data(), W, params_ch)); q.g0_b = b6.add(h0.b); q.g0_w = b6.add(h0.w);
        q.g2_wt = b6.add(transpose64(h2.w.data(), W, W)); q.g2_b = b6.add(h2.b); q.g2_w = b6.add(h2.w);
        const std::vector<double> v1o = cols64(k1.w, W1, IN1, 0, W), v1c = cols64(k1.w, W1, IN1, W, W), v1p = cols64(k1.w, W1, IN1, 2 * W, 27),
                                  v1t = cols64(k1.w, W1, IN1, 2 * W + 27, W);
        q.w1c_wt = b6.add(transpose64(v1c.data(), W1, W)); q.w1c_w = b6.add(v1c);
        q.w1p_wt = b6.add(transpose64(v1p.data(), W1, 27));
        q.w1t_wt = b6.add(transpose64(v1t.data(), W1, W));
        q.b1 = b6.add(k1.b);
        if (kind == 2) {
            q.w1o_wt = b6.add(transpose64(v1o.data(), W1, W));
            Folded64 t0, t2, e0, e2;
            if ((rc = fold_linear64(sd, "time_encoder.0", "", W, W / 2, &t0))) return rc;
            if ((rc = fold_linear64(sd, "time_encoder.2", "", W, W, &t2))) return rc;
            if ((rc = fold_linear64(sd, "object_encoder.0", "", W, object_ch, &e0))) return rc;
            if ((rc = fold_linear64(sd, "object_encoder.2", "", W, W, &e2))) return rc;
            q.te0_wt = b6.add(transpose64(t0.w.data(), W, W / 2)); q.te0_b = b6.add(t0.b);
            q.te2_wt = b6.add(transpose64(t2.w.data(), W, W)); q.te2_b = b6.add(t2.b);
            q.oe0_wt = b6.add(transpose64(e0.w.data(), W, object_ch)); q.oe0_b = b6.add(e0.b);
            q.oe2_wt = b6.add(transpose64(e2.w.data(), W, W)); q.oe2_b = b6.add(e2.b);
        } else {
            Folded64 a0, a1, b0, b1, c0;
            if ((rc = fold_linear64(sd, "object_encoder.sa1.mlp_convs.0", "object_encoder.sa1.mlp_bns.0", 64, 3, &a0))) return rc;
            if ((rc = fold_linear64(sd, "object_encoder.sa1.mlp_convs.1", "object_encoder.sa1.mlp_bns.1", 128, 64, &a1))) return rc;
            if ((rc = fold_linear64(sd, "object_encoder.sa2.mlp_convs.0", "object_encoder.sa2.mlp_bns.0", 128, 131, &b0))) return rc;
            if ((rc = fold_linear64(sd, "object_encoder.sa2.mlp_convs.1", "object_encoder.sa2.mlp_bns.1", 256, 128, &b1))) return rc;
            if ((rc = fold_linear64(sd, "object_encoder.sa3.mlp_convs.0", "object_encoder.sa3.mlp_bns.0", 256, 259, &c0))) return rc;
            q.sa1_w0t = b6.add(transpose64(a0.w.data(), 64, 3)); q.sa1_b0 = b6.add(a0.b);
            q.sa1_w1 = b6.add(a1.w); q.sa1_b1 = b6.add(a1.b);
            q.sa2_wf_t = b6.add(transpose64(cols64(b0.w, 128, 131, 3, 128).data(), 128, 128)); q.sa2_b0 = b6.add(b0.b);
            q.sa2_vx = b6.add(transpose64(cols64(b0.w, 128, 131, 0, 3).data(), 128, 3));
            q.sa2_w1_img = b6.add(pack_mfma64(b1.w.data(), 256, 128)); q.sa2_b1 = b6.add(b1.b);
            q.sa3_w_img = b6.add(pack_mfma64(cols64(c0.w, 256, 259, 3, 256).data(), 256, 256));
            q.sa3_wx = b6.add(transpose64(cols64(c0.w, 256, 259, 0, 3).data(), 256, 3)); q.sa3_b = b6.add(c0.b);
        }
        if ((rc = b6.upload())) return rc;
    }
    *out = m.release();
    return DGDM_OK;
}

extern "C" void dgdm_dynamics_destroy(DgdmDynamics *m) { delete m; }

void DgdmDynamics::fill_trunk(TrunkParams *p) const {
    memset(p, 0, sizeof *p);
    for (int i = 0; i < n_mid; ++i) p->bf[i] = blob.at(off.bf[i]);
    p->n_mid = n_mid;
    p->Wout = blob.at(off.wout); p->bout = blob.at(off.bout);
    p->Wfwd = blob.at4(off.wfwd); p->fwd_bytes = (unsigned)(off.fwd_floats * 4);
    p->Wbwd = blob.at4(off.wbwd); p->bwd_bytes = (unsigned)(off.bwd_floats * 4);
    if (kind == 3) p->b2 = blob.at(off.b2);
}

void DgdmDynamics::fill_trunk_bf16(TrunkParams *p) const {
    p->Wfwd = reinterpret_cast<const float4 *>(static_cast<const char *>(w16.p)); p->fwd_bytes = (unsigned)fwd16_bytes;
    p->Wbwd = reinterpret_cast<const float4 *>(static_cast<const char *>(w16.p) + fwd16_bytes); p->bwd_bytes = (unsigned)bwd16_bytes;
}

void DgdmDynamics::fill_trunk_f16(TrunkParams *p, TrunkF16Scales *sc) const {
    p->Wfwd = reinterpret_cast<const float4 *>(static_cast<const char *>(wf16.p)); p->fwd_bytes = (unsigned)fwdh_bytes;
    p->Wbwd = reinterpret_cast<const float4 *>(static_cast<const char *>(wf16.p) + fwdh_bytes); p->bwd_bytes = (unsigned)bwdh_bytes;
    *sc = f16_scales;
}

PnWeights DgdmDynamics::pn() const {
    PnWeights w{};
    w.r1sq = (float)(0.2 * 0.2);
    w.r2sq = (float)(0.4 * 0.4);
    w.sa1_w0t = blob.at(off.sa1_w0t); w.sa1_b0 = blob.at(off.sa1_b0); w.sa1_w1 = blob.at(off.sa1_w1); w.sa1_b1 = blob.at(off.sa1_b1);
    w.sa2_wf_t = blob.at(off.sa2_wf_t); w.sa2_b0 = blob.at(off.sa2_b0); w.sa2_vx = blob.at(off.sa2_vx);
    w.sa2_w1_img = blob.at4(off.sa2_w1_img); w.sa2_b1 = blob.at(off.sa2_b1);
    w.sa3_w_img16 = reinterpret_cast<const float4 *>(static_cast<const char *>(w16.p) + sa3_16_offset);
    w.sa3_wx = blob.at(off.sa3_wx); w.sa3_b = blob.at(off.sa3_b);
    return w;
}

PnWeights64 DgdmDynamics::pn64() const {
    PnWeights64 w{};
    w.sa1_w0t = blob64.at(off64.sa1_w0t); w.sa1_b0 = blob64.at(off64.sa1_b0); w.sa1_w1 = blob64.at(off64.sa1_w1); w.sa1_b1 = blob64.at(off64.sa1_b1);
    w.sa2_wf_t = blob64.at(off64.sa2_wf_t); w.sa2_b0 = blob64.at(off64.sa2_b0); w.sa2_vx = blob64.at(off64.sa2_vx);
    w.sa2_w1_img = blob64.at(off64.sa2_w1_img); w.sa2_b1 = blob64.at(off64.sa2_b1);
    w.sa3_w_img = blob64.at(off64.sa3_w_img); w.sa3_wx = blob64.at(off64.sa3_wx); w.sa3_b = blob64.at(off64.sa3_b);
    return w;
}

int DgdmDynamics::gripper_forward64(const float *x, int ldx, double *V64, double *genc64, int rows, hipStream_t s) const {
    int rc;
    if ((rc = linear64(x, nullptr, ldx, blob64.at(off64.g0_wt), blob64.at(off64.g0_b), nullptr, 1, V64, nullptr, 256, rows, L, 256, ACT_RELU, s))) return rc;
    return linear64(nullptr, V64, 256, blob64.at(off64.g2_wt), blob64.at(off64.g2_b), nullptr, 1, genc64, nullptr, 256, rows, 256, 256, ACT_NONE, s);
}

int DgdmDynamics::time_part64(float t_scalar, float *tmp , double *tmp64 , double *out64, hipStream_t s) const {
    int rc;
    if ((rc = time_embed(nullptr, t_scalar, blob.at(off.tfreq), tmp, 1, thalf, s))) return rc;
    if (kind == 2) {
        if ((rc = linear64(tmp, nullptr, 2 * thalf, blob64.at(off64.te0_wt), blob64.at(off64.te0_b), nullptr, 1, tmp64, nullptr, 256, 1, 2 * thalf, 256, ACT_SILU, s))) return rc;
        if ((rc = linear64(nullptr, tmp64, 256, blob64.at(off64.te2_wt), blob64.at(off64.te2_b), nullptr, 1, tmp64 + 256, nullptr, 256, 1, 256, 256, ACT_NONE, s))) return rc;
        return linear64(nullptr, tmp64 + 256, 256, blob64.at(off64.w1t_wt), blob64.at(off64.b1), nullptr, 1, out64, nullptr, W1, 1, 256, W1, ACT_NONE, s);
    }
    return linear64(tmp, nullptr, 256, blob64.at(off64.w1t_wt), blob64.at(off64.b1), nullptr, 1, out64, nullptr, W1, 1, 256, W1, ACT_NONE, s);
}

int DgdmDynamics::object_part_2d64(const float *obj, double *tmp64 , double *out64, int n, hipStream_t s) const {
    int rc;
    double *h = tmp64, *e = tmp64 + (size_t)n * 256;
    if ((rc = linear64(obj, nullptr, object_ch, blob64.at(off64.oe0_wt), blob64.at(off64.oe0_b), nullptr, 1, h, nullptr, 256, n, object_ch, 256, ACT_RELU, s))) return rc;
    if ((rc = linear64(nullptr, h, 256, blob64.at(off64.oe2_wt), blob64.at(off64.oe2_b), nullptr, 1, e, nullptr, 256, n, 256, 256, ACT_NONE, s))) return rc;
    return linear64(nullptr, e, 256, blob64.at(off64.w1o_wt), nullptr, nullptr, 1, out64, nullptr, W1, n, 256, W1, ACT_NONE, s);
}

int DgdmDynamics::gripper_forward(const float *x, int ldx, float *V, float *genc, int rows, hipStream_t s) const {
    int rc;
    if ((rc = linear(x, ldx, blob.at(off.g0_wt), blob.at(off.g0_b), nullptr, 1, V, 256, rows, L, 256, ACT_RELU, false, s))) return rc;
    return linear(V, 256, blob.at(off.g2_wt), blob.at(off.g2_b), nullptr, 1, genc, 256, rows, 256, 256, ACT_NONE, false, s);
}

int DgdmDynamics::time_part(const float *t_dev, float t_scalar, float *tmp , float *out, int rows, hipStream_t s) const {
    int rc;
    float *emb = tmp, *h = tmp + (size_t)rows * 256, *enc = tmp + (size_t)rows * 512;
    if ((rc = time_embed(t_dev, t_scalar, blob.at(off.tfreq), emb, rows, thalf, s))) return rc;
    const float *feat = emb;
    if (kind == 2) {
        if ((rc = linear(emb, 2 * thalf, blob.at(off.te0_wt), blob.at(off.te0_b), nullptr, 1, h, 256, rows, 2 * thalf, 256, ACT_SILU, false, s))) return rc;
        if ((rc = linear(h, 256, blob.at(off.te2_wt), blob.at(off.te2_b), nullptr, 1, enc, 256, rows, 256, 256, ACT_NONE, false, s))) return rc;
        feat = enc;
    }
    return linear(feat, 256, blob.at(off.w1t_wt), blob.at(off.b1), nullptr, 1, out, W1, rows, 256, W1, ACT_NONE, false, s);
}

int DgdmDynamics::object_part_2d(const float *obj, float *tmp , float *out, int n, bool accumulate, hipStream_t s) const {
    int rc;
    float *h = tmp, *e = tmp + (size_t)n * 256;
    if ((rc = linear(obj, object_ch, blob.at(off.oe0_wt), blob.at(off.oe0_b), nullptr, 1, h, 256, n, object_ch, 256, ACT_RELU, false, s))) return rc;
    if ((rc = linear(h, 256, blob.at(off.oe2_wt), blob.at(off.oe2_b), nullptr, 1, e, 256, n, 256, 256, ACT_NONE, false, s))) return rc;
    return linear(e, 256, blob.at(off.w1o_wt), nullptr, nullptr, 1, out, W1, n, 256, W1, ACT_NONE, accumulate, s);
}

extern "C" int dgdm_dyn2d_forward(DgdmDynamics *m, const float *x_ctrl, const float *x_ori, const float *x_pos, const float *t,
                                  const float *object, float *logits, int rows, void *stream) {
    DGDM_REQUIRE(m && x_ctrl && x_ori && x_pos && t && object && logits && rows >= 0, DGDM_EINVAL, "dgdm_dyn2d_forward: bad argument");
    if (m->kind != 2) { set_error("model type not supported: dgdm_dyn2d_forward on a 3-D model"); return DGDM_EMODE; }
    if (rows == 0) return DGDM_OK;
    hipStream_t s = (hipStream_t)stream;
    int rc;
    const size_t need = (size_t)rows * (256 + 256 + 32 + 768 + 256) * sizeof(float);
    if ((rc = m->ws.alloc(need))) return rc;
    float *V = m->ws.as<float>(), *genc = V + (size_t)rows * 256, *pose = genc + (size_t)rows * 256, *tmp = pose + (size_t)rows * 32,
          *z1 = tmp + (size_t)rows * 768;
    if ((rc = m->time_part(t, 0.f, tmp, z1, rows, s))) return rc;
    if ((rc = m->object_part_2d(object, tmp, z1, rows, true, s))) return rc;
    if ((rc = m->gripper_forward(x_ctrl, m->L, V, genc, rows, s))) return rc;
    if ((rc = linear(genc, 256, m->blob.at(m->off.w1c_wt), nullptr, nullptr, 1, z1, 256, rows, 256, 256, ACT_NONE, true, s))) return rc;
    if ((rc = pose_embed(x_ori, x_pos, pose, rows, s))) return rc;
    if ((rc = linear(pose, 27, m->blob.at(m->off.w1p_wt), nullptr, nullptr, 1, z1, 256, rows, 27, 256, ACT_NONE, true, s))) return rc;
    TrunkParams p;
    m->fill_trunk(&p);
    p.Atab = z1; p.logits = logits; p.C = rows; p.R = rows; p.xstride = rows; p.B = 1; p.tiles_per_b = 1; p.ntiles = (rows + 31) / 32;
    return trunk_launch(2, true, true, p, s);
}
```

dgdm_amd/csrc/trunk.h:

```cpp
#pragma once
#include "common.h"

namespace dgdm {

struct TrunkObjective {
    float lin[3];
    float quad[3];
    int   use_rowcoef;
    int   pad;
};

struct TrunkParams {
    const float  *bf[8];
    int           n_mid;
    const float4 *Wfwd, *Wbwd;
    unsigned      fwd_bytes, bwd_bytes;
    const float  *Wout;
    const float  *bout;
    const float  *b2;
    const float  *xobj;
    const uint32_t *xobj16;
    const float *const *xtab;
    const uint32_t *const *xtab16;
    const int    *xidx;
    int64_t       xstride;
    const float  *Atab;
    const float  *Ptab;
    const float  *PtabT;
    const float  *Pmax;
    const TrunkObjective *obj;
    const float  *rowcoef;
    const float  *rowfield;
    float        *partial;
    float        *logits;
    int           B, C, tiles_per_b, ntiles;
    int64_t       R;
};

inline double trunk_flops(int kind, const TrunkParams &p, bool rows_mode, bool fwd_only) {
    const double rows = rows_mode ? (double)p.R : (double)(p.ntiles / (p.tiles_per_b > 0 ? p.tiles_per_b : 1)) * p.C;
    const double mid = 2.0 * 256 * 256 * p.n_mid;
    double per_row = (kind == 3) ? (2.0 * 256 * 512 * 2 + mid) : mid;
    if (!fwd_only) per_row += (kind == 3) ? (2.0 * 256 * 512 + mid) : mid;
    return rows * per_row;
}

int trunk_launch(int kind, bool rows_mode, bool fwd_only, const TrunkParams &p, hipStream_t s);

struct TrunkF16Scales {
    int ew_mid[8];
    int ew_l1, ew_l2;
    float l1_norm1;
};
enum class TrunkF16Mode { Grad, Forward, ForwardRowPose };
int trunk_f16l_launch(int kind, TrunkF16Mode mode, const TrunkParams &p, const TrunkF16Scales &sc, hipStream_t s);

int rollout_start(const float *ori_grid, int n_chains, int B, int G, double *state, int32_t *left, double *traj0, hipStream_t s);
int rollout_pose_table(const double *state, const double *w1p_wt, int W1, int n_chains, int B, int G, float *tiles, float *pmax, hipStream_t s);
int rollout_update(const float *logits, const double scale[3], int k, int64_t rows, double *state, int32_t *left, double *traj_next,
                   double *final_state, float *first_logits, hipStream_t s);

int score_tally(const float *logits, int n_chains, int B, int C, const float thr[3], int32_t *counts, float *sums, hipStream_t s);

int objective_values_launch(const float *logits, const TrunkObjective *obj, const float *rowcoef, const float *rowfield, int n_chains, int B, int C,
                            double *values, hipStream_t s);

int label_replicate(const float *fingers, int64_t N, int64_t first, int n_chains, int B, int L, float *dst, hipStream_t s);
int label_tally(const int32_t *counts, const float *sums, int M, int B, int nvalid, int64_t cells, int per_object, float *rows, int64_t row_stride,
                int64_t object_stride, hipStream_t s);
int label_settled(const double *final_state, const int32_t *left, int M, int B, int G, int nvalid, int per_object, double *per_obj, float *rows,
                  int64_t row_stride, int64_t object_stride, hipStream_t s);

int goal_field_build(const float *ori_grid, const float *pos_grid, const float *goals, const DgdmGoalSpec *specs, int n_chains, int B, int G, int P,
                     float *field, hipStream_t s);

int trunk_bf16_launch(int kind, const TrunkParams &p, hipStream_t s);

}
```

dgdm_amd/csrc/trunk_f16l.hip:

```cpp
#include "common.h"
#include <algorithm>
#include "mfma_chain.h"
#include "trunk.h"

namespace dgdm {
namespace f16l {

typedef _Float16 hf16x8_t __attribute__((ext_vector_type(8)));
typedef _Float16 hf16x2_t __attribute__((ext_vector_type(2)));
typedef float hf32x2_t __attribute__((ext_vector_type(2)));
typedef uint32_t hu32x4_t __attribute__((ext_vector_type(4)));

__device__ __forceinline__ f32x16 hmfma(const v4f32 a, const hu32x4_t b, const f32x16 c) {
    return __builtin_amdgcn_mfma_f32_32x32x16_f16(__builtin_bit_cast(hf16x8_t, a), __builtin_bit_cast(hf16x8_t, b), c, 0, 0, 0);
}

__device__ __forceinline__ float pow2f(int e) { return __uint_as_float((uint32_t)(min(max(e, -126), 127) + 127) << 23); }

__device__ __forceinline__ int scale_exp(float m, int lo, int hi) {
    m = fmaxf(m, __shfl_xor(m, 32));
    const int e = (int)((__float_as_uint(m) >> 23) & 0xffu);
    const int k = (m > 0.f && e < 255) ? 12 + 127 - e : 0;
    return min(max(k, lo), hi);
}

__device__ __forceinline__ void split2(float lo, float hi, uint32_t &ph, uint32_t &pl) {
    const hf32x2_t v = {lo, hi};
    const hf16x2_t h = __builtin_convertvector(v, hf16x2_t);
    const hf32x2_t d = v - __builtin_convertvector(h, hf32x2_t);
    ph = __builtin_bit_cast(uint32_t, h);
    pl = __builtin_bit_cast(uint32_t, __builtin_convertvector(d, hf16x2_t));
}
__device__ __forceinline__ void split2_mix(float lo, float hi, uint32_t &ph, uint32_t &pl) {
    uint32_t h, l;
    asm("v_cvt_pk_f16_f32 %0, %1, %2" : "=v"(h) : "v"(lo), "v"(hi));
    asm("v_fma_mixlo_f16 %0, -%1, 1.0, %2 op_sel_hi:[1,0,0]" : "=v"(l) : "v"(h), "v"(lo));
    asm("v_fma_mixhi_f16 %0, -%1, 1.0, %2 op_sel:[1,0,0] op_sel_hi:[1,0,0]" : "+v"(l) : "v"(h), "v"(hi));
    ph = h; pl = l;
}
struct Act2 {
    hu32x4_t v[2][8][2];
};

constexpr int CH = 16, NBUF = 4, AHEAD = NBUF - 2;
constexpr int CQ = CH / 4 , CG = CH / 4 ;
static_assert(NBUF >= 3 && NBUF <= 6 && CQ * AHEAD <= 48, "stream slots: 3 .. 6 (LDS), at most 48 DMA loads in flight per wave (vmcnt)");
typedef __attribute__((address_space(3))) v4f32 lds_f4_t;
__device__ void llvm_amdgcn_raw_buffer_load_lds(wrsrc_t rsrc, __attribute__((address_space(3))) void *lds, int size, int voffset, int soffset, int offset, int aux)
    __asm("llvm.amdgcn.raw.buffer.load.lds");

struct LStream {
    wrsrc_t rs;
    lds_f4_t *buf;
    int voff, wave, lane;
    int base;
    int cur, slot;
    __device__ __forceinline__ void issue(int c) {
        const int sl = c % NBUF;
#pragma unroll
        for (int j = 0; j < CQ; ++j) {
            const int e = CQ * wave + j;
            const uint32_t la = (uint32_t)(uintptr_t)(buf + (sl * CH + e) * 64);
            const int so = base + (c * CH + e) * 1024;
            asm volatile("s_mov_b32 m0, %0\n\ts_nop 0\n\tbuffer_load_dwordx4 %1, %2, %3 offen lds" : : "s"(la), "v"(voff), "s"(rs), "s"(so) : "memory", "m0");
        }
    }
    __device__ __forceinline__ void start(const wrsrc_t rs_, int base_) {
        __builtin_amdgcn_s_barrier();
        rs = rs_; base = base_; cur = 0; slot = 0;
#pragma unroll
        for (int c = 0; c <= AHEAD; ++c) issue(c);
        asm volatile("s_waitcnt vmcnt(%0)" : : "n"(CQ * AHEAD) : "memory");
        __builtin_amdgcn_s_barrier();
    }
    __device__ __forceinline__ void advance() {
        asm volatile("s_waitcnt vmcnt(%0) lgkmcnt(0)" : : "n"(CQ * (AHEAD - 1)) : "memory");
        __builtin_amdgcn_s_barrier();
        issue(cur + AHEAD + 1);
        ++cur;
        slot = slot == NBUF - 1 ? 0 : slot + 1;
    }
    __device__ __forceinline__ v4f32 read(const int e) const { return buf[(slot * CH + e) * 64 + lane]; }
};

#define F16_STEP(accA, accB, w, xh, xl)      \
    do {                                     \
        accA = hmfma(w[1], xh, accA);        \
        accB = hmfma(w[3], xh, accB);        \
        accA = hmfma(w[0], xl, accA);        \
        accB = hmfma(w[2], xl, accB);        \
        accA = hmfma(w[0], xh, accA);        \
        accB = hmfma(w[2], xh, accB);        \
    } while (0)
template <bool FWD, bool BIAS, bool MASKS = true>
__device__ __forceinline__ void stream_layer(LStream &ls, v4f32 (&wn)[4], const lds_f4_t *bias , const f32x16 (&Yp)[8], f32x16 (&Y)[8],
                                             uint32_t (*smask)[256], const int slot_in, const int tid, const int h4, int &E, const int ew) {
    float mx = 0.f;
#pragma unroll
    for (int o = 0; o < 8; ++o)
#pragma unroll
        for (int r = 0; r < 16; ++r) mx = FWD ? fmaxf(mx, Yp[o][r]) : fmaxf(mx, fabsf(Yp[o][r]));
    const int k = scale_exp(mx, -100 - E - ew, 100 - E - ew);
    const float f = pow2f(k);
    E += k + ew;
    const float fb = pow2f(E);
#pragma unroll
    for (int o = 0; o < 8; ++o) {
        if (BIAS) {
#pragma unroll
            for (int q = 0; q < 4; ++q) {
                const v4f32 a = bias[(32 * o + 8 * q + h4) >> 2];
                Y[o][4 * q + 0] = a.x * fb; Y[o][4 * q + 1] = a.y * fb; Y[o][4 * q + 2] = a.z * fb; Y[o][4 * q + 3] = a.w * fb;
            }
        } else {
#pragma unroll
            for (int r = 0; r < 16; ++r) Y[o][r] = 0.f;
        }
    }
    hu32x4_t P[2][2][2];
    uint32_t mk = FWD ? 0u : smask[slot_in][tid];
    auto item = [&](const f32x16 &y, const int blk, const int d, const bool far) __attribute__((always_inline)) {
        const int sh = 2 * d + 16 * (blk & 1);
        float lo, hi;
        if (FWD) {
            const hf32x2_t nv = __builtin_elementwise_fma(hf32x2_t{y[2 * d], y[2 * d + 1]}, hf32x2_t{-f, -f}, hf32x2_t{0.f, 0.f});
            if (MASKS) {
                mk = __builtin_amdgcn_alignbit(mk, __float_as_uint(nv.x), 31);
                mk = __builtin_amdgcn_alignbit(mk, __float_as_uint(nv.y), 31);
            }
            asm("v_max_f32 %0, 0, -%1" : "=v"(lo) : "v"(nv.x));
            asm("v_max_f32 %0, 0, -%1" : "=v"(hi) : "v"(nv.y));
        } else {
            const hf32x2_t v = hf32x2_t{y[2 * d], y[2 * d + 1]} * hf32x2_t{f, f};
            lo = apply_bit(v.x, mk, sh);
            hi = apply_bit(v.y, mk, sh + 1);
        }
        uint32_t a, b;
        if (far) split2_mix(lo, hi, a, b);
        else split2(lo, hi, a, b);
        P[blk & 1][0][d / 4][d % 4] = a; P[blk & 1][1][d / 4][d % 4] = b;
    };
#pragma unroll
    for (int d = 0; d < 8; ++d) item(Yp[0], 0, d, false);
#pragma unroll
    for (int b = 0; b < 8; ++b) {
#pragma unroll
        for (int sx = 0; sx < 2; ++sx) {
#pragma unroll
            for (int pp = 0; pp < 4; ++pp) {
                v4f32 w[4];
#pragma unroll
                for (int j = 0; j < 4; ++j) w[j] = wn[j];
                const int gi = (sx * 4 + pp) & (CG - 1);
                if (gi == CG - 1) ls.advance();
#pragma unroll
                for (int j = 0; j < 4; ++j) wn[j] = ls.read(((gi + 1) & (CG - 1)) * 4 + j);
                if (b < 7) {
                    const int q = sx * 4 + pp, nb = b + 1;
                    if (q == 0 && (nb & 1) == 0) mk = FWD ? 0u : smask[slot_in + nb / 2][tid];
                    item(Yp[nb], nb, q, true);
                    if (MASKS && FWD && q == 7 && (nb & 1) == 1) smask[slot_in + nb / 2][tid] = __builtin_bitreverse32(mk);
                }
                F16_STEP(Y[2 * pp], Y[2 * pp + 1], w, P[b & 1][0][sx], P[b & 1][1][sx]);
                __builtin_amdgcn_sched_barrier(0);
            }
        }
    }
}

template <class Side>
__device__ __forceinline__ f32x16 block_out(LStream &ls, v4f32 (&wn)[4], const Act2 &X, f32x16 za, f32x16 zb, Side &&side) {
#pragma unroll
    for (int ks = 0; ks < 16; ++ks) {
        const int s = (ks & 1) * 2;
        const v4f32 w0 = wn[s], w1 = wn[s + 1];
        if ((ks & (CH / 2 - 1)) == CH / 2 - 2) ls.advance();
        wn[s] = ls.read(((ks + 2) & (CH / 2 - 1)) * 2); wn[s + 1] = ls.read(((ks + 2) & (CH / 2 - 1)) * 2 + 1);
        const hu32x4_t xh = X.v[0][ks / 2][ks % 2], xl = X.v[1][ks / 2][ks % 2];
        side(ks);
        za = hmfma(w1, xh, za);
        zb = hmfma(w0, xl, zb);
        za = hmfma(w0, xh, za);
        __builtin_amdgcn_sched_barrier(0);
    }
#pragma unroll
    for (int r = 0; r < 16; ++r) za[r] += zb[r];
    return za;
}

__device__ __forceinline__ int split_rows(const f32x16 (&Y)[8], Act2 &X) {
    float mx = 0.f;
#pragma unroll
    for (int o = 0; o < 8; ++o)
#pragma unroll
        for (int r = 0; r < 16; ++r) mx = fmaxf(mx, fabsf(Y[o][r]));
    const int k = scale_exp(mx, -100, 100);
    const float f = pow2f(k);
#pragma unroll
    for (int o = 0; o < 8; ++o)
#pragma unroll
        for (int d = 0; d < 8; ++d) {
            uint32_t a, b;
            split2(Y[o][2 * d] * f, Y[o][2 * d + 1] * f, a, b);
            X.v[0][o][d / 4][d % 4] = a; X.v[1][o][d / 4][d % 4] = b;
        }
    return k;
}

__device__ __forceinline__ void rows_sum2(float &a, float &b) {
    asm("s_nop 1\n\t"
        "v_add_f32_dpp %0, %0, %0 quad_perm:[1,0,3,2] row_mask:0xf bank_mask:0xf\n\t"
        "v_add_f32_dpp %1, %1, %1 quad_perm:[1,0,3,2] row_mask:0xf bank_mask:0xf\n\ts_nop 0\n\t"
        "v_add_f32_dpp %0, %0, %0 quad_perm:[2,3,0,1] row_mask:0xf bank_mask:0xf\n\t"
        "v_add_f32_dpp %1, %1, %1 quad_perm:[2,3,0,1] row_mask:0xf bank_mask:0xf\n\ts_nop 0\n\t"
        "v_add_f32_dpp %0, %0, %0 row_half_mirror row_mask:0xf bank_mask:0xf\n\t"
        "v_add_f32_dpp %1, %1, %1 row_half_mirror row_mask:0xf bank_mask:0xf\n\ts_nop 0\n\t"
        "v_add_f32_dpp %0, %0, %0 row_mirror row_mask:0xf bank_mask:0xf\n\t"
        "v_add_f32_dpp %1, %1, %1 row_mirror row_mask:0xf bank_mask:0xf\n\ts_nop 0\n\t"
        "v_add_f32_dpp %0, %0, %0 row_bcast:15 row_mask:0xa bank_mask:0xf\n\t"
        "v_add_f32_dpp %1, %1, %1 row_bcast:15 row_mask:0xa bank_mask:0xf"
        : "+v"(a), "+v"(b));
}

}

using namespace f16l;


template <int KIND, bool FWD_ONLY = false, bool ROWPOSE = false>
__global__ __launch_bounds__(256, 1) void trunk_f16l_kernel(const TrunkParams p, const TrunkF16Scales sc) {
    static_assert(FWD_ONLY || !ROWPOSE, "per-row poses: forward-only kernel");
    constexpr int W1B = (KIND == 3) ? 16 : 8;
    constexpr int W1 = W1B * 32;
    constexpr int NSLOT = (KIND == 3) ? 8 + 7 * 4 : 8 * 4;
    __shared__ uint32_t smask[NSLOT][256];

    const int tid = threadIdx.x;
    const int lane = tid & 63;
    const int wave = __builtin_amdgcn_readfirstlane(tid >> 6);
    __shared__ __attribute__((aligned(16))) v4f32 wbuf[NBUF * CH * 64];
    __shared__ __attribute__((aligned(16))) v4f32 small[(8 * 256 + 768) / 4];
    const bool live = blockIdx.x * 4 + wave < p.ntiles;
    const int tile = min(blockIdx.x * 4 + wave, p.ntiles - 1);
    const int n = lane & 31;
    const int h4 = (lane >> 5) * 4;
    const int voff = lane * 16;

    const int per_chain = p.B * p.tiles_per_b;
    const int chain = tile / per_chain;
    const int rem = tile - chain * per_chain;
    const int b = rem / p.tiles_per_b;
    const int c = (rem - b * p.tiles_per_b) * 32 + n;
    const bool valid = c < p.C;
    const int64_t r = (int64_t)(valid ? c : p.C - 1) * p.B + b;
    const float *arow = p.Atab + (size_t)(chain * p.B + b) * W1;
    const float4 *ptile = reinterpret_cast<const float4 *>(p.PtabT) + (size_t)(ROWPOSE ? tile : rem - b * p.tiles_per_b) * W1B * 4 * 64 + lane;

    f32x16 Y[8];
    uint32_t m[4];
    int slot = 0;
    int E = 0;
    const wrsrc_t rsF = weight_rsrc(p.Wfwd, p.fwd_bytes);
    LStream ls;
    ls.buf = (lds_f4_t *)wbuf; ls.voff = voff; ls.wave = wave; ls.lane = lane;
    v4f32 wn[4];
    if (KIND == 2) {
#pragma unroll
        for (int o = 0; o < 8; ++o) {
#pragma unroll
            for (int q = 0; q < 4; ++q) {
                float4 v = feat4(arow, o, q, h4);
                const float4 w = ptile[(o * 4 + q) * 64];
                Y[o][4 * q + 0] = v.x + w.x; Y[o][4 * q + 1] = v.y + w.y; Y[o][4 * q + 2] = v.z + w.z; Y[o][4 * q + 3] = v.w + w.w;
            }
        }
    } else {
        const float *xrow = p.xtab ? p.xtab[chain] + (size_t)p.xidx[(size_t)chain * p.xstride + r] * 256 : p.xobj + ((size_t)chain * p.xstride + r) * 256;
#pragma unroll
        for (int o = 0; o < 8; ++o) {
#pragma unroll
            for (int q = 0; q < 4; ++q) {
                const float4 v = feat4(xrow, o, q, h4);
                Y[o][4 * q + 0] = v.x; Y[o][4 * q + 1] = v.y; Y[o][4 * q + 2] = v.z; Y[o][4 * q + 3] = v.w;
            }
        }
    }
    for (int i = tid; i < p.n_mid * 64; i += 256) small[i] = *reinterpret_cast<const v4f32 *>(p.bf[i >> 6] + 4 * (i & 63));
    if (tid < 192) small[512 + tid] = *reinterpret_cast<const v4f32 *>(p.Wout + 4 * tid);
    ls.start(rsF, 0);
    const lds_f4_t *sbias = (const lds_f4_t *)small, *swout = (const lds_f4_t *)small + 512;

    if (KIND == 3) {
#pragma unroll
        for (int j = 0; j < 4; ++j) wn[j] = ls.read(j);
        Act2 X;
        const int kx = split_rows(Y, X);
        const float un1 = pow2f(-(kx + sc.ew_l1));
        float am = 0.f;
        {
            const float4 a0 = *reinterpret_cast<const float4 *>(arow + 8 * lane), a1 = *reinterpret_cast<const float4 *>(arow + 8 * lane + 4);
            am = fmaxf(fmaxf(fmaxf(fabsf(a0.x), fabsf(a0.y)), fmaxf(fabsf(a0.z), fabsf(a0.w))), fmaxf(fmaxf(fabsf(a1.x), fabsf(a1.y)), fmaxf(fabsf(a1.z), fabsf(a1.w))));
#pragma unroll
            for (int o = 32; o > 0; o >>= 1) am = fmaxf(am, __shfl_xor(am, o));
        }
        const float zb = am + (ROWPOSE ? p.Pmax[(size_t)tile * 32 + n] : p.Pmax[valid ? c : p.C - 1]) + sc.l1_norm1 * pow2f(13 - kx);
        const int eb = (int)((__float_as_uint(zb) >> 23) & 0xffu);
        const int k2 = (zb > 0.f && eb < 255) ? min(max(12 + 127 - eb, -100), 100) : 0;
        const float f2 = pow2f(k2);
        E = k2 + sc.ew_l2;
        const float fb2 = pow2f(E);
#pragma unroll
        for (int o = 0; o < 8; ++o) {
#pragma unroll
            for (int q = 0; q < 4; ++q) {
                const float4 b4 = feat4(p.b2, o, q, h4);
                Y[o][4 * q + 0] = b4.x * fb2; Y[o][4 * q + 1] = b4.y * fb2; Y[o][4 * q + 2] = b4.z * fb2; Y[o][4 * q + 3] = b4.w * fb2;
            }
        }
        f32x16 zero, tt;
#pragma unroll
        for (int rr = 0; rr < 16; ++rr) zero[rr] = 0.f;
        float4 tv[4], tw[4];
        auto table_terms_request = [&](int kb) __attribute__((always_inline)) {
#pragma unroll
            for (int q = 0; q < 4; ++q) {
                tv[q] = *reinterpret_cast<const float4 *>(arow + 32 * kb + 8 * q + h4);
                tw[q] = ptile[(kb * 4 + q) * 64];
            }
        };
        auto table_terms = [&]() __attribute__((always_inline)) {
#pragma unroll
            for (int q = 0; q < 4; ++q) {
                tt[4 * q + 0] = tv[q].x + tw[q].x; tt[4 * q + 1] = tv[q].y + tw[q].y; tt[4 * q + 2] = tv[q].z + tw[q].z; tt[4 * q + 3] = tv[q].w + tw[q].w;
            }
        };
        table_terms_request(0);
        for (int blk = 0; blk < 16; blk += 2) {
            uint32_t bits2 = 0;
#pragma unroll
            for (int e = 0; e < 2; ++e) {
                const int kb = blk + e;
                f32x16 z = block_out(ls, wn, X, zero, zero, [](int) __attribute__((always_inline)) {});
                table_terms();
                table_terms_request((kb + 1) & 15);
#pragma unroll
                for (int rr = 0; rr < 16; ++rr) z[rr] = fmaf(z[rr], un1, tt[rr]);
                hu32x4_t ah[2], al[2];
#pragma unroll
                for (int d = 0; d < 8; ++d) {
                    float lo = z[2 * d], hi = z[2 * d + 1];
                    const int sh = 2 * d + 16 * e;
                    bits2 |= (lo > 0.f ? 1u : 0u) << sh;
                    bits2 |= (hi > 0.f ? 1u : 0u) << (sh + 1);
                    asm("v_max_f32 %0, 0, %1" : "=v"(lo) : "v"(lo));
                    asm("v_max_f32 %0, 0, %1" : "=v"(hi) : "v"(hi));
                    uint32_t a, bb;
                    split2(lo * f2, hi * f2, a, bb);
                    ah[d / 4][d % 4] = a; al[d / 4][d % 4] = bb;
                }
#pragma unroll
                for (int gq = 0; gq < 8; ++gq) {
                    const int pp = gq / 2, sx = gq % 2;
                    v4f32 w[4];
#pragma unroll
                    for (int j = 0; j < 4; ++j) w[j] = wn[j];
                    if ((gq & (CG - 1)) == CG - 1) ls.advance();
#pragma unroll
                    for (int j = 0; j < 4; ++j) wn[j] = ls.read(((gq + 1) & (CG - 1)) * 4 + j);
                    F16_STEP(Y[2 * pp], Y[2 * pp + 1], w, ah[sx], al[sx]);
                    __builtin_amdgcn_sched_barrier(0);
                }
            }
            if (!FWD_ONLY) smask[blk / 2][tid] = bits2;
        }
        slot = 8;
    }
    if (KIND == 2) {
#pragma unroll
        for (int j = 0; j < 4; ++j) wn[j] = ls.read(j);
    }
    constexpr int BASE = (KIND == 3) ? 8 : 0;
    f32x16 Z[8];
    for (int l = 0; l < p.n_mid; ++l) {
        stream_layer<true, true, !FWD_ONLY>(ls, wn, sbias + 64 * l, Y, Z, smask, BASE + 4 * l, tid, h4, E, sc.ew_mid[l]);
#pragma unroll
        for (int o = 0; o < 8; ++o) Y[o] = Z[o];
    }
    slot = BASE + 4 * p.n_mid;
    relu_mask<8>(Y, m);
    if (!FWD_ONLY) {
#pragma unroll
        for (int i = 0; i < 4; ++i) smask[slot + i][tid] = m[i];
    }
    slot += 4;

    float s0 = 0.f, s1 = 0.f, s2 = 0.f;
#pragma unroll
    for (int o = 0; o < 8; ++o) {
#pragma unroll
        for (int q = 0; q < 4; ++q) {
            const v4f32 w0 = swout[(32 * o + 8 * q + h4) >> 2], w1 = swout[64 + ((32 * o + 8 * q + h4) >> 2)], w2 = swout[128 + ((32 * o + 8 * q + h4) >> 2)];
            const float x0 = Y[o][4 * q + 0], x1 = Y[o][4 * q + 1], x2 = Y[o][4 * q + 2], x3 = Y[o][4 * q + 3];
            s0 = fmaf(w0.w, x3, fmaf(w0.z, x2, fmaf(w0.y, x1, fmaf(w0.x, x0, s0))));
            s1 = fmaf(w1.w, x3, fmaf(w1.z, x2, fmaf(w1.y, x1, fmaf(w1.x, x0, s1))));
            s2 = fmaf(w2.w, x3, fmaf(w2.z, x2, fmaf(w2.y, x1, fmaf(w2.x, x0, s2))));
        }
    }
    s0 += __shfl_xor(s0, 32);
    s1 += __shfl_xor(s1, 32);
    s2 += __shfl_xor(s2, 32);
    const float unE = pow2f(-E);
    const float d0 = fmaf(s0, unE, p.bout[0]), d1 = fmaf(s1, unE, p.bout[1]), d2 = fmaf(s2, unE, p.bout[2]);

    if (FWD_ONLY) {
        asm volatile("s_waitcnt vmcnt(0)" : : : "memory");
        if (live && valid && lane < 32) {
            float *dst = p.logits + ((size_t)chain * p.R + r) * 3;
            dst[0] = d0; dst[1] = d1; dst[2] = d2;
        }
        return;
    }
    const TrunkObjective ob = p.obj[chain];
    const bool rf = ob.use_rowcoef == 2;
    const float *fp = (KIND == 3 || rf) ? p.rowfield + ((size_t)chain * p.R + r) * 3 : p.bout;
    float f0 = 0.f, f1 = 0.f, f2 = 0.f;
    if (KIND == 2) { f0 = fp[0]; f1 = fp[1]; f2 = fp[2]; }
    const wrsrc_t rsB = weight_rsrc(p.Wbwd, p.bwd_bytes);
    ls.start(rsB, 0);
    float g0 = ob.lin[0] + 2.f * ob.quad[0] * d0;
    float g1 = ob.lin[1] + 2.f * ob.quad[1] * d1;
    float g2 = ob.lin[2] + 2.f * ob.quad[2] * d2;
    if (ob.use_rowcoef == 1) g0 = p.rowcoef[(size_t)chain * p.R + r];
    if (KIND == 2) { g0 = rf ? g0 + f0 : g0; g1 = rf ? g1 + f1 : g1; g2 = rf ? g2 + f2 : g2; }
    else if (rf) { g0 += fp[0]; g1 += fp[1]; g2 += fp[2]; }
    if (!valid) { g0 = 0.f; g1 = 0.f; g2 = 0.f; }

#pragma unroll
    for (int o = 0; o < 8; ++o) {
#pragma unroll
        for (int q = 0; q < 4; ++q) {
            const v4f32 w0 = swout[(32 * o + 8 * q + h4) >> 2], w1 = swout[64 + ((32 * o + 8 * q + h4) >> 2)], w2 = swout[128 + ((32 * o + 8 * q + h4) >> 2)];
            Y[o][4 * q + 0] = fmaf(g2, w2.x, fmaf(g1, w1.x, g0 * w0.x));
            Y[o][4 * q + 1] = fmaf(g2, w2.y, fmaf(g1, w1.y, g0 * w0.y));
            Y[o][4 * q + 2] = fmaf(g2, w2.z, fmaf(g1, w1.z, g0 * w0.z));
            Y[o][4 * q + 3] = fmaf(g2, w2.w, fmaf(g1, w1.w, g0 * w0.w));
        }
    }
    E = 0;
#pragma unroll
    for (int j = 0; j < 4; ++j) wn[j] = ls.read(j);

    for (int l = p.n_mid - 1; l >= 0; --l) {
        stream_layer<false, false>(ls, wn, nullptr, Y, Z, smask, BASE + 4 + 4 * l, tid, h4, E, sc.ew_mid[l]);
#pragma unroll
        for (int o = 0; o < 8; ++o) Y[o] = Z[o];
    }
#pragma unroll
    for (int i = 0; i < 4; ++i) m[i] = smask[BASE + i][tid];
    apply_mask<8>(Y, m);

    float *dst = p.partial + (size_t)tile * W1;
    if (KIND == 2) {
        const float un = pow2f(-E);
#pragma unroll
        for (int o = 0; o < 8; ++o) {
#pragma unroll
            for (int q = 0; q < 4; ++q) {
                float4 v;
                v.x = rows_sum(Y[o][4 * q + 0] * un); v.y = rows_sum(Y[o][4 * q + 1] * un);
                v.z = rows_sum(Y[o][4 * q + 2] * un); v.w = rows_sum(Y[o][4 * q + 3] * un);
                if (n == ROWS_SUM_LANE && live) *reinterpret_cast<float4 *>(dst + 32 * o + 8 * q + h4) = v;
            }
        }
    } else {
        Act2 X;
        const int kt = split_rows(Y, X);
        const float un = pow2f(-(E + kt + sc.ew_l2));
        f32x16 zero;
#pragma unroll
        for (int rr = 0; rr < 16; ++rr) zero[rr] = 0.f;
        f32x16 g = block_out(ls, wn, X, zero, zero, [](int) __attribute__((always_inline)) {});
        float4 acc;
        auto fold_one = [&](const int rr, const int kb, const uint32_t bits) __attribute__((always_inline)) {
            if ((rr & 1) == 0) return;
            float a = apply_bit(g[rr - 1] * un, bits, rr - 1), b = apply_bit(g[rr] * un, bits, rr);
            rows_sum2(a, b);
            if (rr % 4 == 1) { acc.x = a; acc.y = b; }
            else {
                acc.z = a; acc.w = b;
                if (n == ROWS_SUM_LANE && live) *reinterpret_cast<float4 *>(dst + 32 * kb + 8 * (rr / 4) + h4) = acc;
            }
        };
        for (int kb = 1; kb < 16; ++kb) {
            const uint32_t bits = smask[(kb - 1) / 2][tid] >> (16 * ((kb - 1) & 1));
            const f32x16 gn = block_out(ls, wn, X, zero, zero, [&](const int ks) __attribute__((always_inline)) { fold_one(ks, kb - 1, bits); });
            g = gn;
        }
        const uint32_t bits = smask[7][tid] >> 16;
#pragma unroll
        for (int rr = 0; rr < 16; ++rr) fold_one(rr, 15, bits);
    }
}

int trunk_f16l_launch(int kind, TrunkF16Mode mode, const TrunkParams &p, const TrunkF16Scales &sc, hipStream_t s) {
    const bool fwd = mode != TrunkF16Mode::Grad, rowpose = mode == TrunkF16Mode::ForwardRowPose;
    if (p.n_mid != (kind == 3 ? 6 : 7) || (fwd && !p.logits) || (rowpose && (!p.PtabT || (kind == 3 && !p.Pmax)))) return DGDM_EINVAL;
    const int grid = (p.ntiles + 3) / 4;
    if (grid == 0) return DGDM_OK;
    void (*kernel)(const TrunkParams, const TrunkF16Scales);
    switch (mode) {
    case TrunkF16Mode::Forward: kernel = kind == 2 ? trunk_f16l_kernel<2, true> : trunk_f16l_kernel<3, true>; break;
    case TrunkF16Mode::ForwardRowPose: kernel = kind == 2 ? trunk_f16l_kernel<2, true, true> : trunk_f16l_kernel<3, true, true>; break;
    default: kernel = kind == 2 ? trunk_f16l_kernel<2> : trunk_f16l_kernel<3>; break;
    }
    prof_begin(s, DGDM_STAGE_TRUNK);
    hipLaunchKernelGGL(kernel, dim3(grid), dim3(256), 0, s, p, sc);
    DGDM_HIP_CHECK(hipGetLastError());
    prof_end(s, DGDM_STAGE_TRUNK, trunk_flops(kind, p, false, fwd));
    return DGDM_OK;
}

}
```

Measured before the change: 20460 samples/s.

## Precompute per-object layer-1 outputs and skip layer 1 in gradient trunk

Adds a per-object table of layer-1 pre-activations (object-feature part times W1), built once per object set by a new kernel. The 3-D gradient trunk kernel gets a TABLED variant that reads these precomputed values plus the pose and time terms instead of streaming layer-1 weights and doing the matmul. It streams a reduced weight image without layer 1. Chains whose objects are not M0-only fall back to the old kernel through a chain list, at the cost of extra memory per object, a table-build kernel, and two launches.

```diff
diff --git a/dgdm_amd/csrc/guidance_api.hip b/dgdm_amd/csrc/guidance_api.hip
--- a/dgdm_amd/csrc/guidance_api.hip
+++ b/dgdm_amd/csrc/guidance_api.hip
@@ -37,6 +37,8 @@
     int    ncr = 0;
     DevBuf Z16, M0_16;
     bool   has16 = false;
+    DevBuf L1Z, L1K;
+    bool   has_l1 = false;
 };
 
 struct PoseGrid {
@@ -81,6 +83,9 @@
     DevBuf labelx, labelcounts, labelsums, labelfinal, labelfirst, labelleft, labelobj;
     int rolltiles_chains = 0;
     DevBuf xidx, xidxchains, xtabptrs;
+    DevBuf l1ptrs, l1objs;
+    bool l1tab = true;
+    int fill_l1ptrs(const std::vector<const ObjectTables *> &of_chain, int *n_tabled, hipStream_t s);
     bool xtab_enabled = true;
     int xtab_policy = 0;
     int grads_since_set = 0;
@@ -142,12 +147,13 @@
     int upload_starts(const int64_t *starts_host, int n_chains, int64_t rows, hipStream_t s, bool need_order = true, int n_calls = 1,
                       int64_t call_stride = 0);
     int ensure_rows(int n_chains, int64_t rows_per_chain);
-    int use_xtab(const int *objidx_host, int n_chains, int64_t rows, bool want16, hipStream_t s);
+    int use_xtab(const int *objidx_host, int n_chains, int64_t rows, bool want16, int *l1, hipStream_t s);
     int build_object(int oi, int slot, hipStream_t s);
     int build_xtab(int oi, hipStream_t s);
-    int run_xobj(const int *objidx_host, int n_chains, int64_t rows, bool want16, bool *used16, bool *via_tab, hipStream_t s);
+    int run_xobj(const int *objidx_host, int n_chains, int64_t rows, bool want16, bool *used16, bool *via_tab, int *l1, hipStream_t s);
     struct Embedded {
         bool tab = false, used16 = false;
+        int l1 = 0;
         int64_t rows_per_chain = 0;
         void point(dgdm::TrunkParams *p, const DgdmGuidance &g, int call, int64_t rows_per_call) const;
     };
@@ -203,6 +209,7 @@
     g->m = model; g->cfg = *cfg;
     g->B = cfg->batch;
     if (const char *e = getenv("DGDM_SERIAL_STEP")) g->serial = atoi(e);
+    if (const char *e = getenv("DGDM_L1TAB")) g->l1tab = atoi(e) != 0;
     const int G = cfg->grid_size, P = cfg->num_pos, C = G * P * P;
     const std::vector<float> lo = linspace_f32(cfg->ori_lo, cfg->ori_hi, G), lp = linspace_f32(-1.f, 1.f, P);
     std::vector<float> ori(C), pos(2 * (size_t)C);
@@ -244,7 +251,8 @@
         g->todo_capacity = (int64_t)nc * R;
         g->pinned_bytes = ((size_t)nc * R * 3 + (size_t)nc * (cfg->num_object_points + 1)) * sizeof(int);
         if ((rc = g->groupoff.alloc((size_t)nc * (cfg->num_object_points + 1) * sizeof(int))) || (rc = g->xidx.alloc((size_t)nc * R * sizeof(int))) ||
-            (rc = g->xidxchains.alloc(sizeof(XidxChain) * nc)) || (rc = g->xtabptrs.alloc(sizeof(void *) * nc)))
+            (rc = g->xidxchains.alloc(sizeof(XidxChain) * nc)) || (rc = g->xtabptrs.alloc(sizeof(void *) * nc)) ||
+            (rc = g->l1ptrs.alloc(sizeof(void *) * 3 * nc)))
             return rc;
         DGDM_HIP_CHECK(hipHostMalloc(&g->pinned, g->pinned_bytes, hipHostMallocDefault));
         DGDM_HIP_CHECK(hipEventCreateWithFlags(&g->pinned_ev, hipEventDisableTiming));
@@ -407,6 +415,19 @@
             (rc = g->pool_F1.alloc(no * N * 128 * 8)) || (rc = g->pool_U.alloc(no * N * 128 * 8)) ||
             (rc = g->pool_fps1t.alloc(no * N * 64 * sizeof(uint4))))
             return rc;
+        const bool l1 = g->l1tab && !g->bf16 && N >= 128;
+        const size_t l1mo = (size_t)std::max(1, g->cfg.max_objects);
+        if (l1) {
+            std::vector<const void *> ptrs(3 * l1mo, nullptr);
+            for (int i = 0; i < (int)g->tables.size(); ++i) {
+                ObjectTables &t = *g->tables[i];
+                if ((rc = t.M0.alloc((size_t)N * 256 * 4)) || (rc = t.L1Z.alloc((size_t)N * 512 * 4)) || (rc = t.L1K.alloc((size_t)N * sizeof(int)))) return rc;
+                ptrs[i] = t.M0.p; ptrs[l1mo + i] = t.L1Z.p; ptrs[2 * l1mo + i] = t.L1K.p;
+            }
+            if ((rc = g->l1objs.alloc(sizeof(void *) * ptrs.size()))) return rc;
+            DGDM_HIP_CHECK(hipMemcpyAsync(g->l1objs.p, ptrs.data(), sizeof(void *) * ptrs.size(), hipMemcpyHostToDevice, s));
+        }
+        for (int i = 0; i < n_objects; ++i) g->tables[i]->has_l1 = l1;
         if (!g->pooled) DGDM_HIP_CHECK(hipEventCreateWithFlags(&g->pooled, hipEventDisableTiming));
         DGDM_HIP_CHECK(hipMemcpyAsync(g->pool_xyz.p, objects_dev, no * N * 3 * 4, hipMemcpyDeviceToDevice, s));
         DGDM_HIP_CHECK(hipEventRecord(g->pooled, s));
@@ -458,6 +479,11 @@
         for (int i = off ? 1 : 0; i < nb; ++i) {
             DGDM_HIP_CHECK(hipEventRecord(g->bev[i], g->bstream[i]));
             DGDM_HIP_CHECK(hipStreamWaitEvent(es, g->bev[i], 0));
+        }
+        if (l1) {
+            void *const *po = g->l1objs.as<void *>();
+            if ((rc = trunk_f16l_l1_tables(reinterpret_cast<const float *const *>(po), g->pool_ncr.as<int>(), reinterpret_cast<float *const *>(po + l1mo),
+                                           reinterpret_cast<int *const *>(po + 2 * l1mo), N, n_objects, g->m->fwdh(), es))) return rc;
         }
         prof_end(s, DGDM_STAGE_TABLES, 0.0);
         const size_t need = no * N + no;
@@ -596,21 +622,44 @@
     return DGDM_OK;
 }
 
-int DgdmGuidance::use_xtab(const int *objidx_host, int n_chains, int64_t rows, bool want16, hipStream_t s) {
+int DgdmGuidance::fill_l1ptrs(const std::vector<const ObjectTables *> &of_chain, int *n_tabled, hipStream_t s) {
+    const int nc = cfg.max_chains;
+    std::vector<const void *> ptrs(3 * (size_t)nc, nullptr);
+    int *list = reinterpret_cast<int *>(ptrs.data() + 2 * (size_t)nc);
+    std::vector<int> rest;
+    int nt = 0;
+    for (size_t i = 0; i < of_chain.size(); ++i) {
+        const ObjectTables *t = of_chain[i];
+        if (!t || !l1tab || !t->has_l1 || t->ncr != 0) { rest.push_back((int)i); continue; }
+        ptrs[i] = t->L1Z.p; ptrs[nc + i] = t->L1K.p;
+        list[nt++] = (int)i;
+    }
+    std::copy(rest.begin(), rest.end(), list + nt);
+    *n_tabled = nt;
+    if (nt) DGDM_HIP_CHECK(hipMemcpyAsync(l1ptrs.p, ptrs.data(), sizeof(void *) * ptrs.size(), hipMemcpyHostToDevice, s));
+    return DGDM_OK;
+}
+
+int DgdmGuidance::use_xtab(const int *objidx_host, int n_chains, int64_t rows, bool want16, int *l1, hipStream_t s) {
     std::vector<XidxChain> xc(n_chains);
     std::vector<const void *> base(n_chains);
+    std::vector<const ObjectTables *> m0_of(n_chains, nullptr);
     for (int i = 0; i < n_chains; ++i) {
         const ObjectTables &t = *tables[objidx_host[i]];
         xc[i].fps1 = t.fps1; xc[i].N = cfg.num_object_points; xc[i].m0_only = t.ncr == 0;
         base[i] = want16 ? (t.ncr == 0 ? (const void *)t.M0_16.p : (const void *)t.X16.p) : (t.ncr == 0 ? (const void *)t.M0.p : (const void *)t.X.p);
-    }
+        if (!want16 && t.ncr == 0) m0_of[i] = &t;
+    }
+    int rc;
+    if ((rc = fill_l1ptrs(m0_of, l1, s))) return rc;
     DGDM_HIP_CHECK(hipMemcpyAsync(xidxchains.p, xc.data(), sizeof(XidxChain) * n_chains, hipMemcpyHostToDevice, s));
     DGDM_HIP_CHECK(hipMemcpyAsync(xtabptrs.p, base.data(), sizeof(void *) * n_chains, hipMemcpyHostToDevice, s));
     return pn_xidx(xidxchains.as<XidxChain>(), starts.as<int>(), rows, n_chains, xidx.as<int>(), s);
 }
 
-int DgdmGuidance::run_xobj(const int *objidx_host, int n_chains, int64_t rows, bool want16, bool *used16, bool *via_tab, hipStream_t s) {
+int DgdmGuidance::run_xobj(const int *objidx_host, int n_chains, int64_t rows, bool want16, bool *used16, bool *via_tab, int *l1, hipStream_t s) {
     *via_tab = false;
+    *l1 = 0;
     std::vector<XobjChain> ch(n_chains);
     for (int i = 0; i < n_chains; ++i) {
         const ObjectTables &t = *tables[objidx_host[i]];
@@ -646,10 +695,12 @@
         std::vector<int> rank;
         std::vector<XidxChain> xc(n_chains);
         std::vector<const void *> base(n_chains);
+        std::vector<const ObjectTables *> m0_of(n_chains, nullptr);
         for (int i = 0; i < n_chains; ++i) {
             const ObjectTables &t = *tables[objidx_host[i]];
             const bool m0_only = by_index && t.ncr == 0 && t.fast_ok;
             if (!m0_only) rank.push_back(i);
+            if (m0_only && !want16) m0_of[i] = &t;
             xc[i].fps1 = m0_only ? t.fps1 : nullptr; xc[i].N = cfg.num_object_points; xc[i].m0_only = 1;
             base[i] = m0_only ? (want16 ? (const void *)t.M0_16.p : (const void *)t.M0.p)
                               : (want16 ? (const void *)(xobj16.as<uint32_t>() + (size_t)i * rows * 128) : (const void *)(xobj.as<float>() + (size_t)i * rows * 256));
@@ -663,6 +714,7 @@
         *via_tab = true;
         DGDM_HIP_CHECK(hipMemcpyAsync(xidxchains.p, xc.data(), sizeof(XidxChain) * n_chains, hipMemcpyHostToDevice, s));
         DGDM_HIP_CHECK(hipMemcpyAsync(xtabptrs.p, base.data(), sizeof(void *) * n_chains, hipMemcpyHostToDevice, s));
+        if ((rc = fill_l1ptrs(m0_of, l1, s))) return rc;
         return pn_xidx(xidxchains.as<XidxChain>(), starts.as<int>(), rows, n_chains, xidx.as<int>(), s);
     }
     return pn_xobj(xp, all_fast, s);
@@ -678,7 +730,7 @@
     if ((rc = upload_starts(starts_host, n_chains, rows_per_call, s, !tab, n_calls, call_stride))) return rc;
     if ((rc = finish_objects())) return rc;
     e->tab = tab; e->used16 = want16; e->rows_per_chain = rt;
-    if ((rc = tab ? use_xtab(oidx, n_chains, rt, want16, s) : run_xobj(oidx, n_chains, rt, want16, &e->used16, &e->tab, s))) return rc;
+    if ((rc = tab ? use_xtab(oidx, n_chains, rt, want16, &e->l1, s) : run_xobj(oidx, n_chains, rt, want16, &e->used16, &e->tab, &e->l1, s))) return rc;
     DGDM_HIP_CHECK(hipEventRecord(up_consumed, s));
     consumed_recorded = true;
     return DGDM_OK;
@@ -691,6 +743,12 @@
         p->xidx = g.xidx.as<int>() + row0;
         if (used16) p->xtab16 = g.xtabptrs.as<const uint32_t *>();
         else p->xtab = g.xtabptrs.as<const float *>();
+        if (l1 && !used16) {
+            p->l1z = g.l1ptrs.as<const float *>();
+            p->l1k = g.l1ptrs.as<const int *>() + g.cfg.max_chains;
+            p->chainlist = reinterpret_cast<const int *>(g.l1ptrs.as<const void *>() + 2 * (size_t)g.cfg.max_chains);
+            p->n_tabled = l1;
+        }
     } else {
         p->xobj = g.xobj.as<float>() + row0 * 256;
         p->xobj16 = used16 ? g.xobj16.as<uint32_t>() + row0 * 128 : nullptr;
diff --git a/dgdm_amd/csrc/models.h b/dgdm_amd/csrc/models.h
--- a/dgdm_amd/csrc/models.h
+++ b/dgdm_amd/csrc/models.h
@@ -53,7 +53,8 @@
     dgdm::DevBuf w16;
     size_t fwd16_bytes = 0, bwd16_bytes = 0, sa3_16_offset = 0;
     dgdm::DevBuf wf16;
-    size_t fwdh_bytes = 0, bwdh_bytes = 0;
+    size_t fwdh_bytes = 0, bwdh_bytes = 0, fwdh_nl1_bytes = 0;
+    const float4 *fwdh() const { return reinterpret_cast<const float4 *>(wf16.p); }
     dgdm::TrunkF16Scales f16_scales{};
     dgdm::DevBuf z1_unit;
 
diff --git a/dgdm_amd/csrc/models_api.hip b/dgdm_amd/csrc/models_api.hip
--- a/dgdm_amd/csrc/models_api.hip
+++ b/dgdm_amd/csrc/models_api.hip
@@ -614,7 +614,20 @@
                 for (int ks = 0; ks < 16; ++ks) st.emit(bs, kb, ks / 2, ks % 2);
         }
         m->fwdh_bytes = fs.size() * 2; m->bwdh_bytes = bs.size() * 2;
+        std::vector<uint16_t> fn;
+        if (kind == 3) {
+            const size_t CHK = 16 * 512;
+            for (int kb = 0; kb < 16; ++kb) fn.insert(fn.end(), fs.begin() + (size_t)(4 * kb + 2) * CHK, fs.begin() + (size_t)(4 * kb + 4) * CHK);
+            fn.insert(fn.end(), fs.begin() + 64 * CHK, fs.end());
+            DGDM_REQUIRE(fn.size() % CHK == 0 && fn.size() + 32 * CHK == fs.size(), DGDM_EINVAL, "f16 split: the stream without layer 1 has the wrong length");
+            for (size_t c = 0; c < fn.size() / CHK; ++c) {
+                const size_t full = c < 32 ? 4 * (c / 2) + 2 + (c & 1) : c + 32;
+                DGDM_REQUIRE(!memcmp(&fn[c * CHK], &fs[full * CHK], CHK * 2), DGDM_EINVAL, "f16 split: chunk %zu of the stream without layer 1 differs from the full stream's", c);
+            }
+        }
+        m->fwdh_nl1_bytes = fn.size() * 2;
         fs.insert(fs.end(), bs.begin(), bs.end());
+        fs.insert(fs.end(), fn.begin(), fn.end());
         if ((rc = m->wf16.upload(fs.data(), fs.size() * 2))) return rc;
     }
     std::vector<float> bwd;
@@ -690,6 +703,8 @@
 void DgdmDynamics::fill_trunk_f16(TrunkParams *p, TrunkF16Scales *sc) const {
     p->Wfwd = reinterpret_cast<const float4 *>(static_cast<const char *>(wf16.p)); p->fwd_bytes = (unsigned)fwdh_bytes;
     p->Wbwd = reinterpret_cast<const float4 *>(static_cast<const char *>(wf16.p) + fwdh_bytes); p->bwd_bytes = (unsigned)bwdh_bytes;
+    p->Wfwd_nl1 = fwdh_nl1_bytes ? reinterpret_cast<const float4 *>(static_cast<const char *>(wf16.p) + fwdh_bytes + bwdh_bytes) : nullptr;
+    p->fwd_nl1_bytes = (unsigned)fwdh_nl1_bytes;
     *sc = f16_scales;
 }
 
diff --git a/dgdm_amd/csrc/trunk.h b/dgdm_amd/csrc/trunk.h
--- a/dgdm_amd/csrc/trunk.h
+++ b/dgdm_amd/csrc/trunk.h
@@ -24,6 +24,13 @@
     const uint32_t *const *xtab16;
     const int    *xidx;
     int64_t       xstride;
+    const float *const *l1z;
+    const int   *const *l1k;
+    const float4 *Wfwd_nl1;
+    unsigned      fwd_nl1_bytes;
+    const int    *chainlist;
+    int           n_tabled;
+    const int    *chains;
     const float  *Atab;
     const float  *Ptab;
     const float  *PtabT;
@@ -54,6 +61,8 @@
 };
 enum class TrunkF16Mode { Grad, Forward, ForwardRowPose };
 int trunk_f16l_launch(int kind, TrunkF16Mode mode, const TrunkParams &p, const TrunkF16Scales &sc, hipStream_t s);
+int trunk_f16l_l1_tables(const float *const *m0, const int *ncr, float *const *l1z, int *const *l1k, int N, int n_objects, const float4 *Wfwd,
+                         hipStream_t s);
 
 int rollout_start(const float *ori_grid, int n_chains, int B, int G, double *state, int32_t *left, double *traj0, hipStream_t s);
 int rollout_pose_table(const double *state, const double *w1p_wt, int W1, int n_chains, int B, int G, float *tiles, float *pmax, hipStream_t s);
diff --git a/dgdm_amd/csrc/trunk_f16l.hip b/dgdm_amd/csrc/trunk_f16l.hip
--- a/dgdm_amd/csrc/trunk_f16l.hip
+++ b/dgdm_amd/csrc/trunk_f16l.hip
@@ -81,6 +81,13 @@
         slot = slot == NBUF - 1 ? 0 : slot + 1;
     }
     __device__ __forceinline__ v4f32 read(const int e) const { return buf[(slot * CH + e) * 64 + lane]; }
+};
+
+struct GStream {
+    const v4f32 *img;
+    int lane, cur;
+    __device__ __forceinline__ void advance() { ++cur; if ((cur & 1) == 0) cur += 2; }
+    __device__ __forceinline__ v4f32 read(const int e) const { return img[((size_t)cur * CH + e) * 64 + lane]; }
 };
 
 #define F16_STEP(accA, accB, w, xh, xl)      \
@@ -168,8 +175,8 @@
     }
 }
 
-template <class Side>
-__device__ __forceinline__ f32x16 block_out(LStream &ls, v4f32 (&wn)[4], const Act2 &X, f32x16 za, f32x16 zb, Side &&side) {
+template <class Stream, class Side>
+__device__ __forceinline__ f32x16 block_out(Stream &ls, v4f32 (&wn)[4], const Act2 &X, f32x16 za, f32x16 zb, Side &&side) {
 #pragma unroll
     for (int ks = 0; ks < 16; ++ks) {
         const int s = (ks & 1) * 2;
@@ -227,9 +234,11 @@
 using namespace f16l;
 
 
-template <int KIND, bool FWD_ONLY = false, bool ROWPOSE = false>
+template <int KIND, bool FWD_ONLY = false, bool ROWPOSE = false, bool TABLED = false>
 __global__ __launch_bounds__(256, 1) void trunk_f16l_kernel(const TrunkParams p, const TrunkF16Scales sc) {
     static_assert(FWD_ONLY || !ROWPOSE, "per-row poses: forward-only kernel");
+    static_assert(!TABLED || (KIND == 3 && !FWD_ONLY), "layer-1 tables: the 3-D gradient kernel");
+    constexpr bool tabled = TABLED;
     constexpr int W1B = (KIND == 3) ? 16 : 8;
     constexpr int W1 = W1B * 32;
     constexpr int NSLOT = (KIND == 3) ? 8 + 7 * 4 : 8 * 4;
@@ -247,8 +256,12 @@
     const int voff = lane * 16;
 
     const int per_chain = p.B * p.tiles_per_b;
-    const int chain = tile / per_chain;
-    const int rem = tile - chain * per_chain;
+    const int cpos = tile / per_chain;
+    const int rem = tile - cpos * per_chain;
+    int chain = cpos, otile = tile;
+    if constexpr (KIND == 3 && !FWD_ONLY) {
+        if (p.chains) { chain = p.chains[cpos]; otile = chain * per_chain + rem; }
+    }
     const int b = rem / p.tiles_per_b;
     const int c = (rem - b * p.tiles_per_b) * 32 + n;
     const bool valid = c < p.C;
@@ -260,7 +273,7 @@
     uint32_t m[4];
     int slot = 0;
     int E = 0;
-    const wrsrc_t rsF = weight_rsrc(p.Wfwd, p.fwd_bytes);
+    const wrsrc_t rsF = tabled ? weight_rsrc(p.Wfwd_nl1, p.fwd_nl1_bytes) : weight_rsrc(p.Wfwd, p.fwd_bytes);
     LStream ls;
     ls.buf = (lds_f4_t *)wbuf; ls.voff = voff; ls.wave = wave; ls.lane = lane;
     v4f32 wn[4];
@@ -274,7 +287,7 @@
                 Y[o][4 * q + 0] = v.x + w.x; Y[o][4 * q + 1] = v.y + w.y; Y[o][4 * q + 2] = v.z + w.z; Y[o][4 * q + 3] = v.w + w.w;
             }
         }
-    } else {
+    } else if (!tabled) {
         const float *xrow = p.xtab ? p.xtab[chain] + (size_t)p.xidx[(size_t)chain * p.xstride + r] * 256 : p.xobj + ((size_t)chain * p.xstride + r) * 256;
 #pragma unroll
         for (int o = 0; o < 8; ++o) {
@@ -294,7 +307,16 @@
 #pragma unroll
         for (int j = 0; j < 4; ++j) wn[j] = ls.read(j);
         Act2 X;
-        const int kx = split_rows(Y, X);
+        int kx;
+        typedef const __attribute__((address_space(1))) float *gfloat_p;
+        gfloat_p zrow = nullptr;
+        if (tabled) {
+            const int tq = p.xidx[(size_t)chain * p.xstride + r];
+            zrow = (gfloat_p)p.l1z[chain] + (size_t)tq * 512;
+            kx = p.l1k[chain][tq];
+        } else {
+            kx = split_rows(Y, X);
+        }
         const float un1 = pow2f(-(kx + sc.ew_l1));
         float am = 0.f;
         {
@@ -334,44 +356,110 @@
                 tt[4 * q + 0] = tv[q].x + tw[q].x; tt[4 * q + 1] = tv[q].y + tw[q].y; tt[4 * q + 2] = tv[q].z + tw[q].z; tt[4 * q + 3] = tv[q].w + tw[q].w;
             }
         };
-        table_terms_request(0);
-        for (int blk = 0; blk < 16; blk += 2) {
-            uint32_t bits2 = 0;
-#pragma unroll
-            for (int e = 0; e < 2; ++e) {
-                const int kb = blk + e;
-                f32x16 z = block_out(ls, wn, X, zero, zero, [](int) __attribute__((always_inline)) {});
-                table_terms();
-                table_terms_request((kb + 1) & 15);
-#pragma unroll
-                for (int rr = 0; rr < 16; ++rr) z[rr] = fmaf(z[rr], un1, tt[rr]);
-                hu32x4_t ah[2], al[2];
-#pragma unroll
-                for (int d = 0; d < 8; ++d) {
-                    float lo = z[2 * d], hi = z[2 * d + 1];
-                    const int sh = 2 * d + 16 * e;
-                    bits2 |= (lo > 0.f ? 1u : 0u) << sh;
-                    bits2 |= (hi > 0.f ? 1u : 0u) << (sh + 1);
-                    asm("v_max_f32 %0, 0, %1" : "=v"(lo) : "v"(lo));
-                    asm("v_max_f32 %0, 0, %1" : "=v"(hi) : "v"(hi));
-                    uint32_t a, bb;
-                    split2(lo * f2, hi * f2, a, bb);
-                    ah[d / 4][d % 4] = a; al[d / 4][d % 4] = bb;
+        auto l1_pair = [&](const f32x16 &z, const int d, const int sh, uint32_t &bits, uint32_t &a, uint32_t &bb) __attribute__((always_inline)) {
+            float lo = z[2 * d], hi = z[2 * d + 1];
+            bits |= (lo > 0.f ? 1u : 0u) << sh;
+            bits |= (hi > 0.f ? 1u : 0u) << (sh + 1);
+            asm("v_max_f32 %0, 0, %1" : "=v"(lo) : "v"(lo));
+            asm("v_max_f32 %0, 0, %1" : "=v"(hi) : "v"(hi));
+            split2(lo * f2, hi * f2, a, bb);
+        };
+        if (!tabled) {
+            table_terms_request(0);
+            for (int blk = 0; blk < 16; blk += 2) {
+                uint32_t bits2 = 0;
+#pragma unroll
+                for (int e = 0; e < 2; ++e) {
+                    const int kb = blk + e;
+                    f32x16 z = block_out(ls, wn, X, zero, zero, [](int) __attribute__((always_inline)) {});
+                    table_terms();
+                    table_terms_request((kb + 1) & 15);
+#pragma unroll
+                    for (int rr = 0; rr < 16; ++rr) z[rr] = fmaf(z[rr], un1, tt[rr]);
+                    hu32x4_t ah[2], al[2];
+#pragma unroll
+                    for (int d = 0; d < 8; ++d) {
+                        uint32_t a, bb;
+                        l1_pair(z, d, 2 * d + 16 * e, bits2, a, bb);
+                        ah[d / 4][d % 4] = a; al[d / 4][d % 4] = bb;
+                    }
+#pragma unroll
+                    for (int gq = 0; gq < 8; ++gq) {
+                        const int pp = gq / 2, sx = gq % 2;
+                        v4f32 w[4];
+#pragma unroll
+                        for (int j = 0; j < 4; ++j) w[j] = wn[j];
+                        if ((gq & (CG - 1)) == CG - 1) ls.advance();
+#pragma unroll
+                        for (int j = 0; j < 4; ++j) wn[j] = ls.read(((gq + 1) & (CG - 1)) * 4 + j);
+                        F16_STEP(Y[2 * pp], Y[2 * pp + 1], w, ah[sx], al[sx]);
+                        __builtin_amdgcn_sched_barrier(0);
+                    }
                 }
-#pragma unroll
-                for (int gq = 0; gq < 8; ++gq) {
-                    const int pp = gq / 2, sx = gq % 2;
-                    v4f32 w[4];
-#pragma unroll
-                    for (int j = 0; j < 4; ++j) w[j] = wn[j];
-                    if ((gq & (CG - 1)) == CG - 1) ls.advance();
-#pragma unroll
-                    for (int j = 0; j < 4; ++j) wn[j] = ls.read(((gq + 1) & (CG - 1)) * 4 + j);
-                    F16_STEP(Y[2 * pp], Y[2 * pp + 1], w, ah[sx], al[sx]);
-                    __builtin_amdgcn_sched_barrier(0);
+                if (!FWD_ONLY) smask[blk / 2][tid] = bits2;
+            }
+        } else if constexpr (!FWD_ONLY) {
+            struct Raw { float4 zv[4], tv[4], tw[4]; } R[2];
+            auto request = [&](Raw &w, const int kb) __attribute__((always_inline)) {
+#pragma unroll
+                for (int q = 0; q < 4; ++q) {
+                    const v4f32 v = *(const __attribute__((address_space(1))) v4f32 *)(zrow + 32 * kb + 8 * q + h4);
+                    w.zv[q] = make_float4(v.x, v.y, v.z, v.w);
+                    w.tv[q] = *reinterpret_cast<const float4 *>(arow + 32 * kb + 8 * q + h4);
+                    w.tw[q] = ptile[(kb * 4 + q) * 64];
                 }
-            }
-            if (!FWD_ONLY) smask[blk / 2][tid] = bits2;
+            };
+            auto take = [&](const Raw &w, f32x16 &z) __attribute__((always_inline)) {
+#pragma unroll
+                for (int q = 0; q < 4; ++q) {
+                    z[4 * q + 0] = fmaf(w.zv[q].x, un1, w.tv[q].x + w.tw[q].x); z[4 * q + 1] = fmaf(w.zv[q].y, un1, w.tv[q].y + w.tw[q].y);
+                    z[4 * q + 2] = fmaf(w.zv[q].z, un1, w.tv[q].z + w.tw[q].z); z[4 * q + 3] = fmaf(w.zv[q].w, un1, w.tv[q].w + w.tw[q].w);
+                }
+            };
+            f32x16 zc[2];
+            hu32x4_t P[2][2][2];
+            uint32_t bits_lo = 0;
+            request(R[0], 0);
+            request(R[1], 1);
+            take(R[0], zc[0]);
+            request(R[0], 2);
+#pragma unroll
+            for (int d = 0; d < 8; ++d) {
+                uint32_t a, bb;
+                l1_pair(zc[0], d, 2 * d, bits_lo, a, bb);
+                P[0][0][d / 4][d % 4] = a; P[0][1][d / 4][d % 4] = bb;
+            }
+            take(R[1], zc[1]);
+            request(R[1], 3);
+#pragma unroll
+            for (int blk = 0; blk < 16; blk += 2) {
+                uint32_t bits_hi = 0, bits_next = 0;
+#pragma unroll
+                for (int e = 0; e < 2; ++e) {
+                    const int kb = blk + e;
+#pragma unroll
+                    for (int gq = 0; gq < 8; ++gq) {
+                        const int pp = gq / 2, sx = gq % 2;
+                        v4f32 w[4];
+#pragma unroll
+                        for (int j = 0; j < 4; ++j) w[j] = wn[j];
+                        if (gq == 3) {
+                            take(R[e], zc[e]);
+                            request(R[e], (kb + 4) & 15);
+                        }
+                        if ((gq & (CG - 1)) == CG - 1) ls.advance();
+#pragma unroll
+                        for (int j = 0; j < 4; ++j) wn[j] = ls.read(((gq + 1) & (CG - 1)) * 4 + j);
+                        uint32_t a, bb;
+                        l1_pair(zc[e ^ 1], gq, 2 * gq + 16 * (e ^ 1), e == 0 ? bits_hi : bits_next, a, bb);
+                        P[e ^ 1][0][gq / 4][gq % 4] = a; P[e ^ 1][1][gq / 4][gq % 4] = bb;
+                        F16_STEP(Y[2 * pp], Y[2 * pp + 1], w, P[e][0][sx], P[e][1][sx]);
+                        __builtin_amdgcn_sched_barrier(0);
+                    }
+                    if (e == 0) smask[blk / 2][tid] = bits_lo | bits_hi;
+                }
+                bits_lo = bits_next;
+            }
         }
         slot = 8;
     }
@@ -459,7 +547,7 @@
     for (int i = 0; i < 4; ++i) m[i] = smask[BASE + i][tid];
     apply_mask<8>(Y, m);
 
-    float *dst = p.partial + (size_t)tile * W1;
+    float *dst = p.partial + (size_t)otile * W1;
     if (KIND == 2) {
         const float un = pow2f(-E);
 #pragma unroll
@@ -502,11 +590,59 @@
     }
 }
 
+__global__ __launch_bounds__(64) void l1_table_kernel(const float *const *m0, const int *ncr, float *const *l1z, int *const *l1k, const int N, const v4f32 *img) {
+    const int obj = blockIdx.y;
+    if (ncr[obj] != 0) return;
+    const int lane = threadIdx.x, n = lane & 31, h4 = (lane >> 5) * 4;
+    const int row = blockIdx.x * 32 + n;
+    const bool valid = row < N;
+    const float *xrow = m0[obj] + (size_t)min(row, N - 1) * 256;
+    f32x16 Y[8];
+#pragma unroll
+    for (int o = 0; o < 8; ++o) {
+#pragma unroll
+        for (int q = 0; q < 4; ++q) {
+            const float4 v = feat4(xrow, o, q, h4);
+            Y[o][4 * q + 0] = v.x; Y[o][4 * q + 1] = v.y; Y[o][4 * q + 2] = v.z; Y[o][4 * q + 3] = v.w;
+        }
+    }
+    Act2 X;
+    const int kx = split_rows(Y, X);
+    if (valid && lane < 32) l1k[obj][row] = kx;
+    GStream gs{img, lane, 0};
+    v4f32 wn[4];
+#pragma unroll
+    for (int j = 0; j < 4; ++j) wn[j] = gs.read(j);
+    f32x16 zero;
+#pragma unroll
+    for (int rr = 0; rr < 16; ++rr) zero[rr] = 0.f;
+    float *dst = l1z[obj] + (size_t)min(row, N - 1) * 512;
+    for (int kb = 0; kb < 16; ++kb) {
+        const f32x16 z = block_out(gs, wn, X, zero, zero, [](int) __attribute__((always_inline)) {});
+        if (valid) {
+#pragma unroll
+            for (int q = 0; q < 4; ++q) *reinterpret_cast<float4 *>(dst + 32 * kb + 8 * q + h4) = make_float4(z[4 * q + 0], z[4 * q + 1], z[4 * q + 2], z[4 * q + 3]);
+        }
+    }
+}
+
+int trunk_f16l_l1_tables(const float *const *m0, const int *ncr, float *const *l1z, int *const *l1k, int N, int n_objects, const float4 *Wfwd,
+                         hipStream_t s) {
+    if (N <= 0 || n_objects <= 0) return DGDM_OK;
+    hipLaunchKernelGGL(l1_table_kernel, dim3((N + 31) / 32, n_objects), dim3(64), 0, s, m0, ncr, l1z, l1k, N, reinterpret_cast<const v4f32 *>(Wfwd));
+    DGDM_HIP_CHECK(hipGetLastError());
+    return DGDM_OK;
+}
+
 int trunk_f16l_launch(int kind, TrunkF16Mode mode, const TrunkParams &p, const TrunkF16Scales &sc, hipStream_t s) {
     const bool fwd = mode != TrunkF16Mode::Grad, rowpose = mode == TrunkF16Mode::ForwardRowPose;
     if (p.n_mid != (kind == 3 ? 6 : 7) || (fwd && !p.logits) || (rowpose && (!p.PtabT || (kind == 3 && !p.Pmax)))) return DGDM_EINVAL;
     const int grid = (p.ntiles + 3) / 4;
     if (grid == 0) return DGDM_OK;
+    const bool split = !fwd && kind == 3 && p.l1z;
+    const int per_chain = p.B * p.tiles_per_b, n_chains = per_chain > 0 ? p.ntiles / per_chain : 0;
+    if (split && (!p.l1k || !p.xtab || !p.xidx || !p.Wfwd_nl1 || !p.chainlist || p.n_tabled < 1 || p.n_tabled > n_chains || n_chains * per_chain != p.ntiles))
+        return DGDM_EINVAL;
     void (*kernel)(const TrunkParams, const TrunkF16Scales);
     switch (mode) {
     case TrunkF16Mode::Forward: kernel = kind == 2 ? trunk_f16l_kernel<2, true> : trunk_f16l_kernel<3, true>; break;
@@ -514,7 +650,19 @@
     default: kernel = kind == 2 ? trunk_f16l_kernel<2> : trunk_f16l_kernel<3>; break;
     }
     prof_begin(s, DGDM_STAGE_TRUNK);
-    hipLaunchKernelGGL(kernel, dim3(grid), dim3(256), 0, s, p, sc);
+    if (split) {
+        TrunkParams q = p;
+        if (p.n_tabled < n_chains) {
+            q.chains = p.chainlist + p.n_tabled; q.ntiles = (n_chains - p.n_tabled) * per_chain;
+            hipLaunchKernelGGL(kernel, dim3((q.ntiles + 3) / 4), dim3(256), 0, s, q, sc);
+        }
+        q.chains = p.chainlist; q.ntiles = p.n_tabled * per_chain;
+        hipLaunchKernelGGL((trunk_f16l_kernel<3, false, false, true>), dim3((q.ntiles + 3) / 4), dim3(256), 0, s, q, sc);
+    } else {
+        TrunkParams q = p;
+        q.chains = nullptr;
+        hipLaunchKernelGGL(kernel, dim3(grid), dim3(256), 0, s, q, sc);
+    }
     DGDM_HIP_CHECK(hipGetLastError());
     prof_end(s, DGDM_STAGE_TRUNK, trunk_flops(kind, p, false, fwd));
     return DGDM_OK;
```

Result: faster. 21180 samples/s, median of 6 (+3.5%).
